# nrclaudio/spVIPES

Measured on AMD Instinct MI355X. Metric: cells/sec/training-step (2-group PoE VAE), higher is better.
Workload: dtype bf16

## Files before the change

include/spvipes_hip.h:

```cpp
#ifndef SPVIPES_HIP_H
#define SPVIPES_HIP_H

#include <stdint.h>

#ifdef __cplusplus
extern "C" {
#endif

#define SPV_OK 0
#define SPV_ERR_ARG (-1)
#define SPV_ERR_LAUNCH (-2)
#define SPV_ERR_UNSUPPORTED (-3)

#define SPV_COUNT_F32 0
#define SPV_COUNT_U16 1

#define SPV_NB_CMAX 64
#define SPV_DEC_KP 16
#define SPV_DEC_KS 32
#define SPV_DEC_KP_WIDE 32
#define SPV_DEC_KS_WIDE 64
#define SPV_DEC_CELLS_PER_WG 128

int spv_version(void);
// ... 252 lines not shown
  int32_t D;
  int32_t k;
  const int32_t* exclude;
  int32_t n_split;
  int32_t* idx; float* dist; int64_t ld_out;
  void* ws;
} spv_knn_args;
int spv_knn(const spv_knn_args* a, void* stream);
int32_t spv_knn_splits(int32_t n_q, int32_t n_c);
int64_t spv_knn_ws_bytes(int32_t n_q, int32_t k, int32_t n_split);
int32_t spv_knn_tile_q(void);
int32_t spv_knn_tile_c(void);

#define SPV_OT_DMAX 64
#define SPV_OT_KMAX 64
#define SPV_OT_SPLIT_MAX 64
typedef struct spv_ot_args {
  const float* Q; int64_t ld_q; int32_t n_q;
  const float* C; int64_t ld_c; int32_t n_c;
  int32_t D;
  int32_t k;
  const float* h;
  const float* r;
  float inv_eps;
  int32_t n_split;
  float* L;
  int32_t* idx; float* val; int64_t ld_out;
  float* mass;
  void* ws;
} spv_ot_args;
int spv_ot_softmin(const spv_ot_args* a, void* stream);
int spv_ot_topk(const spv_ot_args* a, void* stream);
int32_t spv_ot_splits(int32_t n_q, int32_t n_c);
int64_t spv_ot_ws_bytes(int32_t n_q, int32_t k, int32_t n_split);
int32_t spv_ot_tile_q(void);
int32_t spv_ot_tile_c(void);

#define SPV_OT_SEG_MAX 256
typedef struct spv_ot_seg_args {
  const float* Q; int64_t ld_q; int32_t n_q;
  const float* C; int64_t ld_c; int32_t n_c;
  int32_t D;
  const float* h;
  float inv_eps;
  const int32_t* seg_ptr; int32_t n_seg;
  int32_t n_split;
  float* L; int64_t ld_l;
  void* ws;
} spv_ot_seg_args;
int spv_ot_segment_lse(const spv_ot_seg_args* a, void* stream);
int32_t spv_ot_segment_splits(int32_t n_q, int32_t n_c);
int64_t spv_ot_segment_ws_bytes(int32_t n_q, int32_t n_seg, int32_t n_split);

#define SPV_SILHOUETTE_SEG_MAX 256
typedef struct spv_silhouette_args {
  const float* Q; int64_t ld_q; int32_t n_q;
  const float* C; int64_t ld_c; int32_t n_c;
  int32_t D;
  const int32_t* seg_ptr; int32_t n_seg;
  int32_t n_split;
  double* S; int64_t ld_s;
  void* ws;
} spv_silhouette_args;
int spv_silhouette_sums(const spv_silhouette_args* a, void* stream);
int32_t spv_silhouette_splits(int32_t n_q, int32_t n_c);
int64_t spv_silhouette_ws_bytes(int32_t n_q, int32_t n_seg, int32_t n_split);

int spv_dec_dz(const spv_dec_params* p, const float* Tp, const float* Ts, float* dz_part, void* stream);

int spv_dec_softmax_bwd(const spv_dec_params* p, const float* Tp, const float* Ts, float* dz_part, void* stream);
int spv_dec_heads_bwd(const spv_dec_params* p, const float* Tp, const float* Ts, float* dz_part, float* dw_part, void* stream);

#define SPV_ADAM_MAX_IMAGES 16
#define SPV_IMAGE_BF16 0
#define SPV_IMAGE_F16 1
typedef struct spv_adam_image {
  int64_t begin, count;
  int32_t cols, row_off, col_off, fmt;
  int64_t ld;
  uint16_t* dst;
  float scale; int32_t _pad;
} spv_adam_image;

int spv_adam_step_images(float* p, const float* g, float* m, float* v, int64_t n, float lr, float beta1, float beta2, float eps,
                         float weight_decay, float bc1, float bc2, float grad_scale, const spv_adam_image* images, int32_t n_images,
                         int64_t* step_counter, const int64_t* t_dev, double beta1_d, double beta2_d, void* stream);

typedef struct spv_gather_prob { const uint32_t* src; const int32_t* idx; uint32_t* dst; int64_t count; } spv_gather_prob;
int spv_gather_u32(const spv_gather_prob* probs, int32_t nprob, void* stream);

int spv_randn(float* out, int64_t n, const int64_t* counter, uint64_t key, void* stream);
int spv_counter_bump(int64_t* counter, void* stream);

int spv_adam_step(float* p, const float* g, float* m, float* v, int64_t n, float lr, float beta1,
                  float beta2, float eps, float weight_decay, float bc1, float bc2, float grad_scale,
                  void* stream);

#define SPV_MAXP 8

typedef struct spv_linear_prob {
  const float* X; int64_t ldx;
  const float* W;
  const float* bias;
  float* Y; int64_t ldy;
  const float* dY; int64_t lddy;
  float* dX; int64_t lddx;
  float* dW; float* db;
  int32_t N, K;
  const float* keep;
  const float* W2; int32_t n_w2;
  uint16_t* img_hi; uint16_t* img_lo; int64_t ld_img; int32_t img_rows;
} spv_linear_prob;
typedef struct spv_linear_batch {
  spv_linear_prob p[SPV_MAXP];
  int32_t nprob, B;
  int32_t relu;
  float drop_p;
  uint64_t seed;
  const uint64_t* seed_ptr;
  int32_t accumulate;
} spv_linear_batch;
int spv_linear_fwd(const spv_linear_batch* a, void* stream);
int spv_linear_dgrad(const spv_linear_batch* a, void* stream);
int spv_linear_wgrad(const spv_linear_batch* a, float* wpart, int64_t wpart_elems, void* stream);

typedef struct spv_linear_pending_prob { float* dW; float* db; int32_t N, K; } spv_linear_pending_prob;
typedef struct spv_linear_pending {
  spv_linear_pending_prob p[SPV_MAXP];
  int32_t nprob;
  const float* wpart; int64_t prob_stride;
} spv_linear_pending;
int spv_linear_bwd(const spv_linear_batch* d, const spv_linear_batch* w, float* wpart, int64_t wpart_elems,
                   const spv_linear_pending* pending, void* stream);
int spv_linear_reduce_pending(const spv_linear_pending* pending, void* stream);

typedef struct spv_bn_prob {
  const float* X; int64_t ldx;
  float* Y; int64_t ldy;
  const float* gamma; const float* beta;
  float* running_mean; float* running_var;
  float* stats;
  float* part;
  const float* dY; int64_t lddy;
  float* dX; int64_t lddx;
  float* dgamma; float* dbeta;
  int32_t N;
  uint16_t* img_hi; uint16_t* img_lo; int64_t ld_img; int32_t img_rows;
} spv_bn_prob;
typedef struct spv_bn_batch {
  spv_bn_prob p[SPV_MAXP];
  int32_t nprob, B, training, relu;
  float eps, momentum;
} spv_bn_batch;
int spv_bn_fwd(const spv_bn_batch* a, void* stream);
int spv_bn_bwd(const spv_bn_batch* a, void* stream);

typedef struct spv_sample_prob {
  const float* post; int32_t n;
  const float* eps;
  float* scale; float* logz; float* theta; float* kl;
  const float* g_loc; const float* g_logvar; const float* g_scale; const float* g_logz; const float* g_kl;
  float* d_post;
  int64_t g_ld;
} spv_sample_prob;
typedef struct spv_sample_batch { spv_sample_prob p[SPV_MAXP]; int32_t nprob, B; } spv_sample_batch;
int spv_enc_sample_fwd(const spv_sample_batch* a, void* stream);
int spv_enc_sample_bwd(const spv_sample_batch* a, void* stream);
int spv_enc_heads_fwd(const spv_bn_batch* bn, const spv_sample_batch* sb, void* stream);
int spv_enc_heads_bwd(const spv_bn_batch* bn, const spv_sample_batch* sb, void* stream);
// ... 45 lines not shown
} spv_poe_comp_args;
int spv_poe_comp_fwd(const spv_poe_comp_args* a, void* stream);
int spv_poe_comp_bwd(const spv_poe_comp_args* a, void* stream);

typedef struct spv_plan {
  const int32_t* ptr0; const int32_t* ind0; const float* val0; int32_t n0;
  const int32_t* ptr1; const int32_t* ind1; const float* val1; int32_t n1;
} spv_plan;
int spv_plan_invmap(const int32_t* idx0, int32_t B0, const int32_t* idx1, int32_t B1, int32_t* inv0, int32_t n0, int32_t* inv1,
                    int32_t n1, void* stream);
typedef struct spv_plan_expert_args {
  spv_plan plan;
  const int32_t* idx[2]; const int32_t* inv[2]; const float* comp[2];
  const float* stats[2]; int64_t ld[2];
  float* expert[2]; int64_t ld_expert[2];
  float* rowsum[2];
  const float* d_expert[2]; float* d_stats[2];
  int32_t B, n;
} spv_plan_expert_args;
int spv_plan_expert_fwd(const spv_plan_expert_args* a, void* stream);
int spv_plan_expert_bwd(const spv_plan_expert_args* a, void* stream);
int spv_plan_argmax(const spv_plan* plan, const int32_t* idx0, const int32_t* idx1, const int32_t* inv0, const int32_t* inv1,
                    int32_t B0, int32_t B1, int32_t* partner0, int32_t* partner1, void* stream);

typedef struct spv_zsplit_args {
  const float* priv[2]; const float* poe[2];
  float* zcat[2];
  const float* d_zcat[2]; float* d_priv[2]; float* d_poe[2];
  int32_t B, n_p, n_s, ngroups;
  uint16_t* am_hi[2]; uint16_t* am_lo[2]; int64_t ld_am; int32_t am_col; int32_t am_cols;
  uint16_t* aps_hi[2]; uint16_t* aps_lo[2]; int32_t Bp;
  int32_t kslots;
} spv_zsplit_args;
int spv_zsplit_fwd(const spv_zsplit_args* a, void* stream);
int spv_zsplit_bwd(const spv_zsplit_args* a, void* stream);

typedef struct spv_fold_prob {
  const float* W; const float* gamma; const float* beta;
  float* running_mean; float* running_var;
  const float* zsum; const float* zz;
  const float* z; int64_t ldz;
  float* stat;
  uint16_t* img_hi; uint16_t* img_lo; int64_t ld_img; int32_t col_off; int32_t slot;
  const float* dWeff; int64_t ld_dw;
  float* dW; float* dgamma; float* dbeta;
  float* red_part;
  float* dz; int64_t lddz;
  int32_t G, Gp, K;
  int32_t zcol; float* out_priv; float* out_poe; int32_t n_p, n_s;
} spv_fold_prob;
typedef struct spv_fold_batch {
  spv_fold_prob p[SPV_MAXP]; int32_t nprob, B, training; float eps, momentum;
  int32_t kslots;
} spv_fold_batch;
int spv_bn_fold_fwd(const spv_fold_batch* a, void* stream);
int spv_bn_fold_bwd(const spv_fold_batch* a, void* stream);

#define SPV_TRUNK_KMAX 48
typedef struct spv_trunk_prob {
  const float* W; const float* bias; const float* gamma; const float* beta;
  float* running_mean; float* running_var;
  const float* zsum; const float* zz;
  float* Wf; float* cf; float* stat;
  const float* dWf; const float* dcf;
  float* dW; float* dbias; float* dgamma; float* dbeta;
  float* dred;
  const float* z; int64_t ldz; float* dz; int64_t lddz;
  int32_t N, K;
} spv_trunk_prob;
typedef struct spv_trunk_batch { spv_trunk_prob p[2]; int32_t nprob, B, training; float eps, momentum; } spv_trunk_batch;
int spv_trunk_fold_fwd(const spv_trunk_batch* a, void* stream);
int spv_trunk_fold_bwd(const spv_trunk_batch* a, void* stream);

#define SPV_MAXR 16
typedef struct spv_reduce_prob {
  const float* src; int64_t slab_stride; int64_t ld_src; int32_t nslabs; int32_t col_off;
  int32_t rows, cols;
  float* dst; int64_t ld_dst; int32_t accumulate; int32_t pad_;
  const float* alpha; const float* exp_scale;
} spv_reduce_prob;
typedef struct spv_reduce_batch { spv_reduce_prob p[SPV_MAXR]; int32_t nprob; } spv_reduce_batch;
int spv_reduce_slabs(const spv_reduce_batch* b, void* stream);

int spv_loss_assemble(const float* rec0, const float* rec1, const float* w, const float* const* kl, int32_t nkl, int32_t B,
                      const float* kl_weight, float* loss, float* rec_sum, float* gkl, void* stream);

#ifdef __cplusplus
}
#endif
#endif
```

spvipes_amd/_abi.py:

```python
from __future__ import annotations

import ctypes as C
import os
from typing import NamedTuple, Optional

import torch

_HERE = os.path.dirname(os.path.abspath(__file__))
LIB_PATH = os.path.join(_HERE, "_lib", "libspvipes_hip.so")

SPV_COUNT_F32, SPV_COUNT_U16 = 0, 1
NB_CMAX, DEC_KP, DEC_KS, DEC_CELLS_PER_WG = 64, 16, 32, 128
DEC_KPS = DEC_KP + DEC_KS


class DecSlots(NamedTuple):
    kslots: int
    KP: int
    KS: int
    KPS: int


DEC_NARROW = DecSlots(0, DEC_KP, DEC_KS, DEC_KPS)
DEC_WIDE = DecSlots(1, 32, 64, 96)
# ... 46 lines not shown
                ("N", C.c_int32), ("K", C.c_int32), ("keep", C.c_void_p), ("W2", C.c_void_p), ("n_w2", C.c_int32),
                ("img_hi", C.c_void_p), ("img_lo", C.c_void_p), ("ld_img", C.c_int64), ("img_rows", C.c_int32)]


class SpvLinearBatch(C.Structure):
    _fields_ = [("p", SpvLinearProb * SPV_MAXP), ("nprob", C.c_int32), ("B", C.c_int32), ("relu", C.c_int32), ("drop_p", C.c_float),
                ("seed", C.c_uint64), ("seed_ptr", C.c_void_p), ("accumulate", C.c_int32)]


class SpvLinearPendingProb(C.Structure):
    _fields_ = [("dW", C.c_void_p), ("db", C.c_void_p), ("N", C.c_int32), ("K", C.c_int32)]


class SpvLinearPending(C.Structure):
    _fields_ = [("p", SpvLinearPendingProb * SPV_MAXP), ("nprob", C.c_int32), ("wpart", C.c_void_p), ("prob_stride", C.c_int64)]


class SpvBnProb(C.Structure):
    _fields_ = [("X", C.c_void_p), ("ldx", C.c_int64), ("Y", C.c_void_p), ("ldy", C.c_int64), ("gamma", C.c_void_p), ("beta", C.c_void_p),
                ("running_mean", C.c_void_p), ("running_var", C.c_void_p), ("stats", C.c_void_p), ("part", C.c_void_p),
                ("dY", C.c_void_p), ("lddy", C.c_int64), ("dX", C.c_void_p), ("lddx", C.c_int64), ("dgamma", C.c_void_p), ("dbeta", C.c_void_p),
                ("N", C.c_int32), ("img_hi", C.c_void_p), ("img_lo", C.c_void_p), ("ld_img", C.c_int64), ("img_rows", C.c_int32)]


class SpvBnBatch(C.Structure):
    _fields_ = [("p", SpvBnProb * SPV_MAXP), ("nprob", C.c_int32), ("B", C.c_int32), ("training", C.c_int32), ("relu", C.c_int32),
                ("eps", C.c_float), ("momentum", C.c_float)]


class SpvSampleProb(C.Structure):
    _fields_ = [("post", C.c_void_p), ("n", C.c_int32), ("eps", C.c_void_p), ("scale", C.c_void_p), ("logz", C.c_void_p), ("theta", C.c_void_p),
                ("kl", C.c_void_p), ("g_loc", C.c_void_p), ("g_logvar", C.c_void_p), ("g_scale", C.c_void_p), ("g_logz", C.c_void_p),
                ("g_kl", C.c_void_p), ("d_post", C.c_void_p), ("g_ld", C.c_int64)]


class SpvSampleBatch(C.Structure):
    _fields_ = [("p", SpvSampleProb * SPV_MAXP), ("nprob", C.c_int32), ("B", C.c_int32)]


class SpvPoeArgs(C.Structure):
    _fields_ = [("stats", C.c_void_p * 2), ("ld", C.c_int64 * 2), ("partner", C.c_void_p * 2), ("mode", C.c_void_p * 2), ("eps", C.c_void_p * 2),
                ("loc", C.c_void_p * 2), ("logvar", C.c_void_p * 2), ("scale", C.c_void_p * 2), ("logz", C.c_void_p * 2), ("theta", C.c_void_p * 2),
                ("kl", C.c_void_p * 2), ("g_loc", C.c_void_p * 2), ("g_logvar", C.c_void_p * 2), ("g_scale", C.c_void_p * 2),
                ("g_logz", C.c_void_p * 2), ("g_kl", C.c_void_p * 2), ("d_stats", C.c_void_p * 2), ("B", C.c_int32 * 2), ("n", C.c_int32),
                ("clamp_scale", C.c_int32), ("lone_passthrough", C.c_int32), ("expert", C.c_void_p * 2), ("ld_expert", C.c_int64 * 2),
                ("d_expert", C.c_void_p * 2), ("lab", C.c_void_p * 2), ("order", C.c_void_p * 2), ("rank", C.c_void_p * 2), ("tables", C.c_void_p)]


SPV_POE_MAXG, POE_COMP_SEG, POE_COMP_CMAX = 4, 16, 64


class SpvFc1FwdArgs(C.Structure):
    _fields_ = [("x", C.POINTER(SpvCounts)), ("B", C.c_int32), ("G", C.c_int32), ("W1_hi", C.c_void_p), ("W1_lo", C.c_void_p), ("ldw", C.c_int64),
                ("N1", C.c_int32), ("bias", C.c_void_p), ("bias2", C.c_void_p), ("n_first", C.c_int32), ("nsplit", C.c_int32), ("splits", C.c_int32),
                ("slabs", C.c_void_p), ("rowsum_ws", C.c_void_p), ("h1", C.c_void_p), ("library", C.c_void_p), ("xb_all", C.c_void_p),
                ("ld_xb", C.c_int64), ("library_all", C.c_void_p), ("cov", C.c_void_p), ("cov_idx", C.c_void_p)]


class SpvFc1BwdArgs(C.Structure):
    _fields_ = [("dh1", C.c_void_p), ("h1", C.c_void_p), ("x", C.POINTER(SpvCounts)), ("B", C.c_int32), ("G", C.c_int32), ("N1", C.c_int32),
                ("n_first", C.c_int32), ("nsplit", C.c_int32), ("Bp", C.c_int32), ("dh_hi", C.c_void_p), ("dh_lo", C.c_void_p), ("ld_dh", C.c_int64),
                ("part", C.c_void_p), ("db", C.c_void_p), ("db2", C.c_void_p), ("dW", C.c_void_p), ("dW2", C.c_void_p), ("ldc", C.c_int64),
                ("xb", C.c_void_p), ("ld_xb", C.c_int64), ("scale_ws", C.c_void_p)]


class SpvGatherProb(C.Structure):
    _fields_ = [("src", C.c_void_p), ("idx", C.c_void_p), ("dst", C.c_void_p), ("count", C.c_int64)]


def gather_u32(probs) -> None:
    arr = (SpvGatherProb * len(probs))()
    for a, (src, idx, dst) in zip(arr, probs):
        a.src, a.idx, a.dst, a.count = ptr(src), ptr(idx), ptr(dst), dst.numel()
    call("spv_gather_u32", arr, len(probs), stream_ptr())


ADAM_MAX_IMAGES = 16
IMAGE_BF16, IMAGE_F16 = 0, 1


class SpvAdamImage(C.Structure):
    _fields_ = [("begin", C.c_int64), ("count", C.c_int64), ("cols", C.c_int32), ("row_off", C.c_int32), ("col_off", C.c_int32), ("fmt", C.c_int32),
                ("ld", C.c_int64), ("dst", C.c_void_p), ("scale", C.c_float), ("_pad", C.c_int32)]


class SpvPoeCompArgs(C.Structure):
    _fields_ = ([("ngroups", C.c_int32), ("n", C.c_int32), ("ncomp", C.c_int32), ("pad_", C.c_int32), ("B", C.c_int32 * SPV_POE_MAXG),
                 ("stats", C.c_void_p * SPV_POE_MAXG), ("ld", C.c_int64 * SPV_POE_MAXG), ("comp", C.c_void_p * SPV_POE_MAXG),
                 ("eps", C.c_void_p * SPV_POE_MAXG), ("part", C.c_void_p), ("mean", C.c_void_p)]
                + [(k, C.c_void_p * SPV_POE_MAXG) for k in ("loc", "logvar", "scale", "logz", "theta", "kl", "g_loc", "g_logvar", "g_scale", "g_logz", "g_kl",
                                                            "dpn", "d_stats")])


class SpvPlan(C.Structure):
    _fields_ = [("ptr0", C.c_void_p), ("ind0", C.c_void_p), ("val0", C.c_void_p), ("n0", C.c_int32),
                ("ptr1", C.c_void_p), ("ind1", C.c_void_p), ("val1", C.c_void_p), ("n1", C.c_int32)]


class SpvPlanExpertArgs(C.Structure):
    _fields_ = [("plan", SpvPlan), ("idx", C.c_void_p * 2), ("inv", C.c_void_p * 2), ("comp", C.c_void_p * 2), ("stats", C.c_void_p * 2),
                ("ld", C.c_int64 * 2), ("expert", C.c_void_p * 2), ("ld_expert", C.c_int64 * 2), ("rowsum", C.c_void_p * 2),
                ("d_expert", C.c_void_p * 2), ("d_stats", C.c_void_p * 2), ("B", C.c_int32), ("n", C.c_int32)]


class SpvZsplitArgs(C.Structure):
    _fields_ = [("priv", C.c_void_p * 2), ("poe", C.c_void_p * 2), ("zcat", C.c_void_p * 2), ("d_zcat", C.c_void_p * 2),
                ("d_priv", C.c_void_p * 2), ("d_poe", C.c_void_p * 2), ("B", C.c_int32), ("n_p", C.c_int32), ("n_s", C.c_int32), ("ngroups", C.c_int32),
                ("am_hi", C.c_void_p * 2), ("am_lo", C.c_void_p * 2), ("ld_am", C.c_int64), ("am_col", C.c_int32), ("am_cols", C.c_int32),
                ("aps_hi", C.c_void_p * 2), ("aps_lo", C.c_void_p * 2), ("Bp", C.c_int32), ("kslots", C.c_int32)]


class SpvFoldProb(C.Structure):
    _fields_ = [("W", C.c_void_p), ("gamma", C.c_void_p), ("beta", C.c_void_p), ("running_mean", C.c_void_p), ("running_var", C.c_void_p),
                ("zsum", C.c_void_p), ("zz", C.c_void_p), ("z", C.c_void_p), ("ldz", C.c_int64), ("stat", C.c_void_p),
                ("img_hi", C.c_void_p), ("img_lo", C.c_void_p), ("ld_img", C.c_int64), ("col_off", C.c_int32), ("slot", C.c_int32),
                ("dWeff", C.c_void_p), ("ld_dw", C.c_int64), ("dW", C.c_void_p), ("dgamma", C.c_void_p), ("dbeta", C.c_void_p),
                ("red_part", C.c_void_p), ("dz", C.c_void_p), ("lddz", C.c_int64), ("G", C.c_int32), ("Gp", C.c_int32), ("K", C.c_int32),
                ("zcol", C.c_int32), ("out_priv", C.c_void_p), ("out_poe", C.c_void_p), ("n_p", C.c_int32), ("n_s", C.c_int32)]


class SpvFoldBatch(C.Structure):
    _fields_ = [("p", SpvFoldProb * SPV_MAXP), ("nprob", C.c_int32), ("B", C.c_int32), ("training", C.c_int32), ("eps", C.c_float),
                ("momentum", C.c_float), ("kslots", C.c_int32)]


class SpvGemmFixup(C.Structure):
    _fields_ = [("counters", C.c_void_p), ("alpha", C.c_void_p), ("dst0", C.c_void_p), ("ld0", C.c_int64), ("n0", C.c_int32),
                ("dst1", C.c_void_p), ("ld1", C.c_int64), ("c1", C.c_int32), ("n1", C.c_int32)]


class SpvGemmArgs(C.Structure):
    _fields_ = [("a_kmajor", C.c_int32), ("pad0_", C.c_int32), ("A_hi", C.c_void_p), ("A_lo", C.c_void_p), ("lda", C.c_int64),
                ("B_hi", C.c_void_p), ("B_lo", C.c_void_p), ("ldb", C.c_int64), ("C", C.c_void_p), ("ldc", C.c_int64),
                ("M", C.c_int32), ("N", C.c_int32), ("K", C.c_int32), ("nsplit", C.c_int32), ("splits", C.c_int32), ("a_tiles", C.c_int32),
                ("slab_stride", C.c_int64)]


class SpvDecGroup(C.Structure):
    _fields_ = [("p", SpvDecParams), ("library", C.c_void_p), ("px_r", C.c_void_p),
                ("Am_hi", C.c_void_p), ("Am_lo", C.c_void_p), ("Wm_hi", C.c_void_p), ("Wm_lo", C.c_void_p), ("K", C.c_int32), ("nsplit", C.c_int32),
                ("Tp", C.c_void_p), ("Ts", C.c_void_p), ("dz_part", C.c_void_p), ("dw_part", C.c_void_p)]


class SpvDecExpectedArgs(C.Structure):
    _fields_ = [("Am_hi", C.c_void_p), ("Am_lo", C.c_void_p), ("Wm_hi", C.c_void_p), ("Wm_lo", C.c_void_p), ("K", C.c_int32), ("nsplit", C.c_int32),
                ("genes", C.c_void_p), ("n_genes", C.c_int32), ("what", C.c_int32), ("out", C.c_void_p), ("ld_out", C.c_int64),
                ("alpha", C.c_float), ("accumulate", C.c_int32)]


class SpvDecSampleArgs(C.Structure):
    _fields_ = [("Am_hi", C.c_void_p), ("Am_lo", C.c_void_p), ("Wm_hi", C.c_void_p), ("Wm_lo", C.c_void_p), ("K", C.c_int32), ("nsplit", C.c_int32),
                ("genes", C.c_void_p), ("n_genes", C.c_int32), ("ld_gene", C.c_int32), ("theta", C.c_void_p), ("cell_ids", C.c_void_p),
                ("key", C.c_uint64), ("sample", C.c_uint32), ("out", C.c_void_p), ("ld_out", C.c_int64)]


class SpvDecSampleStatsArgs(C.Structure):
    _fields_ = [("Am_hi", C.c_void_p), ("Am_lo", C.c_void_p), ("Wm_hi", C.c_void_p), ("Wm_lo", C.c_void_p), ("K", C.c_int32), ("nsplit", C.c_int32),
                ("genes", C.c_void_p), ("n_genes", C.c_int32), ("n_seg", C.c_int32), ("theta", C.c_void_p), ("cell_ids", C.c_void_p),
                ("key", C.c_uint64), ("sample", C.c_uint32), ("seg", C.c_void_p), ("stats", C.c_void_p), ("ld_stats", C.c_int64),
                ("cell_total", C.c_void_p)]


class SpvDecExpectedStatsArgs(C.Structure):
    _fields_ = [("Am_hi", C.c_void_p), ("Am_lo", C.c_void_p), ("Wm_hi", C.c_void_p), ("Wm_lo", C.c_void_p), ("K", C.c_int32), ("nsplit", C.c_int32),
                ("genes", C.c_void_p), ("n_genes", C.c_int32), ("n_seg", C.c_int32), ("tile_seg", C.c_void_p), ("tile_n", C.c_void_p),
                ("stats", C.c_void_p), ("ld_stats", C.c_int64), ("ws", C.c_void_p)]
# ... 109 lines not shown
    "spv_dec_lse": (C.c_int, [C.POINTER(SpvDecParams), C.c_void_p, C.c_void_p]),
    "spv_dec_nb_fwd": (C.c_int, [C.POINTER(SpvDecParams), C.c_int32, C.c_void_p]),
    "spv_dec_logits": (C.c_int, [C.c_void_p, C.c_void_p, C.c_void_p, C.c_void_p, C.c_int32, C.c_int32, C.c_int32, C.c_int32,
                                 C.c_void_p, C.c_int32, C.c_void_p]),
    "spv_dec_materialize": (C.c_int, [C.POINTER(SpvDecParams), C.c_void_p, C.c_void_p, C.c_void_p, C.c_void_p, C.c_void_p, C.c_int64, C.c_void_p]),
    "spv_dec_expected": (C.c_int, [C.POINTER(SpvDecParams), C.POINTER(SpvDecExpectedArgs), C.c_void_p]),
    "spv_dec_sample": (C.c_int, [C.POINTER(SpvDecParams), C.POINTER(SpvDecSampleArgs), C.c_void_p]),
    "spv_dec_sample_stats": (C.c_int, [C.POINTER(SpvDecParams), C.POINTER(SpvDecSampleStatsArgs), C.c_void_p]),
    "spv_dec_expected_stats": (C.c_int, [C.POINTER(SpvDecParams), C.POINTER(SpvDecExpectedStatsArgs), C.c_void_p]),
    "spv_dec_expected_stats_ws_bytes": (C.c_int64, [C.c_int32, C.c_int32]),
    "spv_nbmix_sample": (C.c_int, [C.c_void_p, C.c_void_p, C.c_void_p, C.c_int64, C.c_void_p, C.c_int32, C.c_int32, C.c_void_p, C.c_uint64, C.c_uint32,
                                   C.c_void_p, C.c_int64, C.c_void_p]),
    "spv_de_pairs": (C.c_int, [C.POINTER(SpvDePairsArgs), C.c_void_p]),
    "spv_de_pairs_splits": (C.c_int32, [C.c_int32, C.c_int32]),
    "spv_de_median": (C.c_int, [C.POINTER(SpvDeMedianArgs), C.c_void_p]),
    "spv_de_median_ws_bytes": (C.c_int64, [C.c_int32, C.c_int32]),
    "spv_count_stats": (C.c_int, [C.POINTER(SpvCountStatsArgs), C.c_void_p]),
    "spv_count_stats_partial": (C.c_int, [C.POINTER(SpvCountStatsArgs), C.c_void_p]),
    "spv_count_stats_merge": (C.c_int, [C.POINTER(SpvCountStatsArgs), C.c_void_p]),
    "spv_count_stats_tile": (C.c_int32, []),
    "spv_count_stats_slab": (C.c_int32, []),
    "spv_count_stats_ws_bytes": (C.c_int64, [C.c_int32, C.c_int32]),
    "spv_count_totals": (C.c_int, [C.POINTER(SpvCounts), C.c_int32, C.c_int32, C.c_void_p, C.c_void_p]),
    "spv_csr_totals": (C.c_int, [C.c_void_p, C.c_void_p, C.c_void_p, C.c_int32, C.c_int32, C.c_int32, C.c_void_p, C.c_void_p]),
    "spv_knn": (C.c_int, [C.POINTER(SpvKnnArgs), C.c_void_p]),
    "spv_knn_splits": (C.c_int32, [C.c_int32, C.c_int32]),
    "spv_knn_ws_bytes": (C.c_int64, [C.c_int32, C.c_int32, C.c_int32]),
    "spv_knn_tile_q": (C.c_int32, []),
    "spv_knn_tile_c": (C.c_int32, []),
    "spv_ot_softmin": (C.c_int, [C.POINTER(SpvOtArgs), C.c_void_p]),
    "spv_ot_topk": (C.c_int, [C.POINTER(SpvOtArgs), C.c_void_p]),
    "spv_ot_splits": (C.c_int32, [C.c_int32, C.c_int32]),
    "spv_ot_ws_bytes": (C.c_int64, [C.c_int32, C.c_int32, C.c_int32]),
    "spv_ot_tile_q": (C.c_int32, []),
    "spv_ot_tile_c": (C.c_int32, []),
    "spv_ot_segment_lse": (C.c_int, [C.POINTER(SpvOtSegArgs), C.c_void_p]),
    "spv_ot_segment_splits": (C.c_int32, [C.c_int32, C.c_int32]),
    "spv_ot_segment_ws_bytes": (C.c_int64, [C.c_int32, C.c_int32, C.c_int32]),
    "spv_silhouette_sums": (C.c_int, [C.POINTER(SpvSilhouetteArgs), C.c_void_p]),
    "spv_silhouette_splits": (C.c_int32, [C.c_int32, C.c_int32]),
    "spv_silhouette_ws_bytes": (C.c_int64, [C.c_int32, C.c_int32, C.c_int32]),
    "spv_dec_dz": (C.c_int, [C.POINTER(SpvDecParams), C.c_void_p, C.c_void_p, C.c_void_p, C.c_void_p]),
    "spv_dec_softmax_bwd": (C.c_int, [C.POINTER(SpvDecParams), C.c_void_p, C.c_void_p, C.c_void_p, C.c_void_p]),
    "spv_dec_heads_bwd": (C.c_int, [C.POINTER(SpvDecParams), C.c_void_p, C.c_void_p, C.c_void_p, C.c_void_p, C.c_void_p]),
    "spv_dec_tables_grouped": (C.c_int, [C.POINTER(SpvDecGroup), C.c_int32, C.c_void_p]),
    "spv_dec_logits_grouped": (C.c_int, [C.POINTER(SpvDecGroup), C.c_int32, C.c_void_p]),
    "spv_dec_lse_grouped": (C.c_int, [C.POINTER(SpvDecGroup), C.c_int32, C.c_void_p]),
    "spv_dec_nb_fwd_grouped": (C.c_int, [C.POINTER(SpvDecGroup), C.c_int32, C.c_int32, C.c_void_p]),
    "spv_dec_heads_bwd_grouped": (C.c_int, [C.POINTER(SpvDecGroup), C.c_int32, C.c_void_p]),
    "spv_gemm_bf16_grouped": (C.c_int, [C.POINTER(SpvGemmArgs), C.c_int32, C.c_void_p]),
    "spv_linear_fwd": (C.c_int, [C.POINTER(SpvLinearBatch), C.c_void_p]),
    "spv_linear_dgrad": (C.c_int, [C.POINTER(SpvLinearBatch), C.c_void_p]),
    "spv_linear_wgrad": (C.c_int, [C.POINTER(SpvLinearBatch), C.c_void_p, C.c_int64, C.c_void_p]),
    "spv_linear_bwd": (C.c_int, [C.POINTER(SpvLinearBatch), C.POINTER(SpvLinearBatch), C.c_void_p, C.c_int64, C.POINTER(SpvLinearPending), C.c_void_p]),
    "spv_linear_reduce_pending": (C.c_int, [C.POINTER(SpvLinearPending), C.c_void_p]),
    "spv_bn_fwd": (C.c_int, [C.POINTER(SpvBnBatch), C.c_void_p]),
    "spv_bn_bwd": (C.c_int, [C.POINTER(SpvBnBatch), C.c_void_p]),
    "spv_enc_sample_fwd": (C.c_int, [C.POINTER(SpvSampleBatch), C.c_void_p]),
    "spv_enc_sample_bwd": (C.c_int, [C.POINTER(SpvSampleBatch), C.c_void_p]),
    "spv_enc_heads_fwd": (C.c_int, [C.POINTER(SpvBnBatch), C.POINTER(SpvSampleBatch), C.c_void_p]),
    "spv_enc_heads_bwd": (C.c_int, [C.POINTER(SpvBnBatch), C.POINTER(SpvSampleBatch), C.c_void_p]),
    "spv_poe_partner": (C.c_int, [C.c_void_p, C.c_void_p, C.c_int32, C.c_int32, C.c_void_p, C.c_void_p, C.c_void_p, C.c_void_p, C.c_void_p,
                                  C.c_void_p, C.c_void_p, C.c_void_p, C.c_void_p, C.c_void_p, C.c_void_p]),
    "spv_poe_rank": (C.c_int, [C.c_void_p, C.c_void_p, C.c_int32, C.c_int32, C.c_void_p, C.c_void_p, C.c_void_p, C.c_void_p, C.c_void_p, C.c_void_p, C.c_void_p]),
    "spv_poe_fuse_fwd": (C.c_int, [C.POINTER(SpvPoeArgs), C.c_void_p]),
    "spv_poe_fuse_bwd": (C.c_int, [C.POINTER(SpvPoeArgs), C.c_void_p]),
    "spv_plan_invmap": (C.c_int, [C.c_void_p, C.c_int32, C.c_void_p, C.c_int32, C.c_void_p, C.c_int32, C.c_void_p, C.c_int32, C.c_void_p]),
    "spv_plan_argmax": (C.c_int, [C.POINTER(SpvPlan), C.c_void_p, C.c_void_p, C.c_void_p, C.c_void_p, C.c_int32, C.c_int32, C.c_void_p,
                                  C.c_void_p, C.c_void_p]),
    "spv_plan_expert_fwd": (C.c_int, [C.POINTER(SpvPlanExpertArgs), C.c_void_p]),
    "spv_plan_expert_bwd": (C.c_int, [C.POINTER(SpvPlanExpertArgs), C.c_void_p]),
    "spv_poe_comp_fwd": (C.c_int, [C.POINTER(SpvPoeCompArgs), C.c_void_p]),
    "spv_poe_comp_bwd": (C.c_int, [C.POINTER(SpvPoeCompArgs), C.c_void_p]),
    "spv_zsplit_fwd": (C.c_int, [C.POINTER(SpvZsplitArgs), C.c_void_p]),
    "spv_zsplit_bwd": (C.c_int, [C.POINTER(SpvZsplitArgs), C.c_void_p]),
    "spv_bn_fold_fwd": (C.c_int, [C.POINTER(SpvFoldBatch), C.c_void_p]),
    "spv_bn_fold_bwd": (C.c_int, [C.POINTER(SpvFoldBatch), C.c_void_p]),
    "spv_trunk_fold_fwd": (C.c_int, [C.POINTER(SpvTrunkBatch), C.c_void_p]),
    "spv_trunk_fold_bwd": (C.c_int, [C.POINTER(SpvTrunkBatch), C.c_void_p]),
    "spv_reduce_slabs": (C.c_int, [C.POINTER(SpvReduceBatch), C.c_void_p]),
    "spv_loss_assemble": (C.c_int, [C.c_void_p, C.c_void_p, C.c_void_p, C.POINTER(C.c_void_p), C.c_int32, C.c_int32, C.c_void_p, C.c_void_p,
                                    C.c_void_p, C.c_void_p, C.c_void_p]),
    "spv_adam_step_images": (C.c_int, [C.c_void_p, C.c_void_p, C.c_void_p, C.c_void_p, C.c_int64, C.c_float, C.c_float, C.c_float, C.c_float,
                                       C.c_float, C.c_float, C.c_float, C.c_float, C.c_void_p, C.c_int32, C.c_void_p, C.c_void_p, C.c_double, C.c_double,
                                       C.c_void_p]),
    "spv_gather_u32": (C.c_int, [C.c_void_p, C.c_int32, C.c_void_p]),
    "spv_randn": (C.c_int, [C.c_void_p, C.c_int64, C.c_void_p, C.c_uint64, C.c_void_p]),
    "spv_counter_bump": (C.c_int, [C.c_void_p, C.c_void_p]),
    "spv_adam_step": (C.c_int, [C.c_void_p, C.c_void_p, C.c_void_p, C.c_void_p, C.c_int64, C.c_float, C.c_float, C.c_float,
                                C.c_float, C.c_float, C.c_float, C.c_float, C.c_float, C.c_void_p]),
}

EXPORTED_SYMBOLS = tuple(_SIGNATURES)
_lib = None


class SpvError(RuntimeError):
    pass


def load() -> C.CDLL:
    global _lib
    if _lib is not None:
        return _lib
    if not os.path.exists(LIB_PATH):
        raise SpvError(
            f"{LIB_PATH} is missing: build it with `python -m spvipes_amd.build` (hipcc, gfx950). "
            "spvipes_amd has no CPU or eager-PyTorch fallback for the hot path."
        )
    lib = C.CDLL(LIB_PATH)
    for name, (res, args) in _SIGNATURES.items():
        fn = getattr(lib, name)
        fn.restype, fn.argtypes = res, args
    from .build import build_id

    have, want = (lib.spv_build_id() or b"").decode(), build_id()
    if have != want and os.environ.get("SPV_ALLOW_STALE_LIB", "0") != "1":
        raise SpvError(f"{LIB_PATH} is stale (built from fingerprint {have}, the sources and flags now give {want}): "
                       "rebuild with `python -m spvipes_amd.build`")
    _lib = lib
    return lib


def check(rc: int, what: str) -> None:
    if rc != 0:
        msg = load().spv_last_error()
        raise SpvError(f"{what} failed with code {rc}: {msg.decode() if msg else ''}")


_PROFILE = None


def profile_start(names) -> None:
    global _PROFILE
    _PROFILE = {n: [] for n in names}


def profile_stop() -> dict:
    global _PROFILE
    prof, _PROFILE = _PROFILE or {}, None
    torch.cuda.synchronize()
    return {n: [s.elapsed_time(e) for s, e in evs] for n, evs in prof.items()}


def call(name: str, *args) -> None:
    fn = getattr(load(), name)
    if _PROFILE is not None and name in _PROFILE:
        s, e = torch.cuda.Event(enable_timing=True), torch.cuda.Event(enable_timing=True)
        s.record()
        rc = fn(*args)
        e.record()
        _PROFILE[name].append((s, e))
    else:
        rc = fn(*args)
    check(rc, name)


def stream_ptr() -> int:
    return torch.cuda.current_stream().cuda_stream


def ptr(t: Optional[torch.Tensor]) -> Optional[int]:
    if t is None:
        return None
    if not t.is_cuda:
        raise SpvError("spvipes_amd kernels need tensors resident in HBM (got a CPU tensor)")
    return t.data_ptr()

# ... 4 lines not shown
```

spvipes_amd/build.py:

```python
from __future__ import annotations

import os
import shutil
import subprocess
import sys

HERE = os.path.dirname(os.path.abspath(__file__))
CSRC = os.path.join(HERE, "csrc")
LIBDIR = os.path.join(HERE, "_lib")
LIB = os.path.join(LIBDIR, "libspvipes_hip.so")
SOURCES = ["spv_abi.hip"]
HEADERS = ["spv_common.h", "spv_gemm.h", "spv_fc1.h", "spv_dec_gemm.h", "spv_decoder.h", "spv_dec_expected.h", "spv_dec_sample.h", "spv_dec_sample_stats.h", "spv_dec_expected_stats.h", "spv_de.h", "spv_de_median.h", "spv_count_stats.h", "spv_knn.h", "spv_pair_scan.h", "spv_ot.h", "spv_ot_segments.h", "spv_silhouette.h", "spv_small.h", "spv_poe_n.h", os.path.join("..", "..", "include", "spvipes_hip.h")]


FLAGS = [
    "--offload-arch=gfx950", "-O3", "-std=c++17", "-fPIC", "-shared", "-Wno-unused-value",
    "-fno-slp-vectorize",
]


def build_id() -> str:
    import hashlib

    h = hashlib.sha256()
    h.update(" ".join(FLAGS).encode())
    for name in sorted(SOURCES + HEADERS):
        with open(os.path.join(CSRC, name), "rb") as f:
            h.update(name.replace(os.sep, "/").encode() + b"\0" + f.read())
    return h.hexdigest()[:32]


def _hipcc() -> str:
    for cand in (os.environ.get("HIPCC"), shutil.which("hipcc"), "/opt/rocm/bin/hipcc"):
        if cand and os.path.exists(cand):
            return cand
    raise RuntimeError("hipcc not found (need ROCm >= 7 with gfx950 support)")


def lib_build_id(path: str = LIB) -> str:
    import re

    if not os.path.exists(path):
        return ""
    with open(path, "rb") as f:
        m = re.search(rb"SPV_BUILD_ID=([0-9a-f]{32})", f.read())
    return m.group(1).decode() if m else ""


def is_stale() -> bool:
    return lib_build_id() != build_id()


def build(force: bool = False, verbose: bool = True) -> str:
    if not force and not is_stale():
        return LIB
    os.makedirs(LIBDIR, exist_ok=True)
    cmd = [
        _hipcc(), *FLAGS, f'-DSPV_BUILD_ID="{build_id()}"',
        *[os.path.join(CSRC, s) for s in SOURCES], "-o", LIB + ".tmp",
    ]
    if verbose:
        print("[spvipes_amd.build]", " ".join(cmd), flush=True)
    subprocess.run(cmd, check=True, cwd=CSRC)
    os.replace(LIB + ".tmp", LIB)
    return LIB


if __name__ == "__main__":
    build(force="--force" in sys.argv)
    print(LIB)
```

spvipes_amd/csrc/spv_abi.hip:

```cpp
#include "../../include/spvipes_hip.h"
#include "spv_common.h"
#include "spv_gemm.h"
#include "spv_fc1.h"
#include "spv_dec_gemm.h"
#include "spv_decoder.h"
#include "spv_dec_expected.h"
#include "spv_dec_sample.h"
#include "spv_dec_sample_stats.h"
#include "spv_dec_expected_stats.h"
#include "spv_de.h"
#include "spv_de_median.h"
#include "spv_count_stats.h"
#include "spv_knn.h"
#include "spv_ot.h"
#include "spv_ot_segments.h"
#include "spv_silhouette.h"
#include "spv_small.h"
#include "spv_poe_n.h"

#include <cstdio>
#include <cstdlib>
#include <cstring>
#include <type_traits>

// ... 1141 lines not shown
  if (dtype == SPV_COUNT_U16) hipLaunchKernelGGL((csr_totals_kernel<true>), grid, block, 0, (hipStream_t)stream, (const long*)indptr, cols, vals, n_cells, G, total);
  else if (dtype == SPV_COUNT_F32) hipLaunchKernelGGL((csr_totals_kernel<false>), grid, block, 0, (hipStream_t)stream, (const long*)indptr, cols, vals, n_cells, G, total);
  else return fail(SPV_ERR_ARG, "spv_csr_totals: unknown count dtype%s");
  return launch_status("spv_csr_totals");
}

extern "C" int spv_dec_dz(const spv_dec_params* q, const float* Tp, const float* Ts, float* dz_part, void* stream) {
  DecParams p;
  int rc = to_dec(q, p);
  if (rc != SPV_OK) return rc;
  if (!Tp || !Ts || !p.tP || !p.tS || !p.lse_p || !p.lse_s || !dz_part) return fail(SPV_ERR_ARG, "spv_dec_dz: null pointer%s");
  if (p.n_gene_tiles != p.Gp / 32) return fail(SPV_ERR_ARG, "spv_dec_dz: n_gene_tiles must be Gp / 32%s");
  if (p.grads_f32) return fail(SPV_ERR_UNSUPPORTED, "spv_dec_dz: needs bf16 gradient arrays%s");
  if (dec_kw(q) != 1) return fail(SPV_ERR_UNSUPPORTED, "spv_dec_dz: narrow operand layout only (kslots = 0)%s");
  hipLaunchKernelGGL((dec_softmax_bwd_kernel<bf16_t, true, false>), dim3(p.Bp / DEC_CELLS_PER_WG, p.gene_splits), dim3(256), 0, (hipStream_t)stream, p, Tp, Ts, dz_part, (float*)nullptr, (float*)nullptr);
  return launch_status("spv_dec_dz");
}

extern "C" int spv_dec_softmax_bwd(const spv_dec_params* q, const float* Tp, const float* Ts, float* dz_part, void* stream) {
  DecParams p;
  int rc = to_dec(q, p);
  if (rc != SPV_OK) return rc;
  if (!Tp || !Ts || !p.tP || !p.tS || !p.lse_p || !p.lse_s) return fail(SPV_ERR_ARG, "spv_dec_softmax_bwd: null pointer%s");
  if (p.n_gene_tiles != p.Gp / 32) return fail(SPV_ERR_ARG, "spv_dec_softmax_bwd: n_gene_tiles must be Gp / 32%s");
  dim3 grid(p.Bp / DEC_CELLS_PER_WG, p.gene_splits);
  hipStream_t s = (hipStream_t)stream;
  float* const none = nullptr;
  if (dec_kw(q) == 2) {
    if (dz_part) return fail(SPV_ERR_UNSUPPORTED, "spv_dec_softmax_bwd: the wide operand layout (kslots = 1) takes no dz_part%s");
    if (p.grads_f32) hipLaunchKernelGGL((dec_softmax_bwd_kernel<split_t, false, true, false, 2>), grid, dim3(256), 0, s, p, Tp, Ts, none, none, none);
    else hipLaunchKernelGGL((dec_softmax_bwd_kernel<bf16_t, false, true, false, 2>), grid, dim3(256), 0, s, p, Tp, Ts, none, none, none);
    return launch_status("spv_dec_softmax_bwd");
  }
  if (p.grads_f32 && dz_part) hipLaunchKernelGGL((dec_softmax_bwd_kernel<split_t, true>), grid, dim3(256), 0, s, p, Tp, Ts, dz_part, none, none);
  else if (p.grads_f32) hipLaunchKernelGGL((dec_softmax_bwd_kernel<split_t, false>), grid, dim3(256), 0, s, p, Tp, Ts, none, none, none);
  else if (dz_part) hipLaunchKernelGGL((dec_softmax_bwd_kernel<bf16_t, true>), grid, dim3(256), 0, s, p, Tp, Ts, dz_part, none, none);
  else hipLaunchKernelGGL((dec_softmax_bwd_kernel<bf16_t, false>), grid, dim3(256), 0, s, p, Tp, Ts, none, none, none);
  return launch_status("spv_dec_softmax_bwd");
}

static int heads_bwd_prepare(const spv_dec_params* q, const float* Tp, const float* Ts, const float* dz_part, const float* dw_part, DecParams& p) {
  int rc = to_dec(q, p);
  if (rc != SPV_OK) return rc;
  if (!Tp || !Ts || !p.tP || !p.tS || !p.lse_p || !p.lse_s || !dz_part || !dw_part) return fail(SPV_ERR_ARG, "spv_dec_heads_bwd: null pointer%s");
  if (p.n_gene_tiles != p.Gp / 32) return fail(SPV_ERR_ARG, "spv_dec_heads_bwd: n_gene_tiles must be Gp / 32%s");
  if (p.Bp % DEC_CELLS_PER_WG) return fail(SPV_ERR_ARG, "spv_dec_heads_bwd: Bp must be a multiple of 128%s");
  if (p.grads_f32 && (!p.Wps_lo || !p.Aps_lo)) return fail(SPV_ERR_ARG, "spv_dec_heads_bwd: split gradient words need the lo planes of the operand images%s");
  if (dec_kw(q) != 1) return fail(SPV_ERR_UNSUPPORTED, "spv_dec_heads_bwd: narrow operand layout only (kslots = 0)%s");
  return SPV_OK;
}
extern "C" int spv_dec_heads_bwd(const spv_dec_params* q, const float* Tp, const float* Ts, float* dz_part, float* dw_part, void* stream) {
  DecParams p;
  int rc = heads_bwd_prepare(q, Tp, Ts, dz_part, dw_part, p);
  if (rc != SPV_OK) return rc;
  dim3 grid(p.Bp / DEC_CELLS_PER_WG, p.gene_splits);
  if (p.grads_f32) {
    launch_lds<dec_heads_bwd_split_kernel>(grid, dim3(256), HBS_LDS_BYTES, (hipStream_t)stream, p, Tp, Ts, dz_part, dw_part);
    return launch_status("spv_dec_heads_bwd");
  }
  hipLaunchKernelGGL(dec_heads_bwd_kernel, grid, dim3(256), 0, (hipStream_t)stream, p, Tp, Ts, dz_part, dw_part);
  return launch_status("spv_dec_heads_bwd");
}
extern "C" int spv_dec_heads_bwd_grouped(const spv_dec_group* g, int32_t n, void* stream) {
  if (!g || n <= 0) return fail(SPV_ERR_ARG, "spv_dec_heads_bwd_grouped: bad arguments%s");
  return pairs_then_rest(n,
    [&](int i) {
      HeadsBwdArgs a0, a1;
      int rc = heads_bwd_prepare(&g[i].p, g[i].Tp, g[i].Ts, g[i].dz_part, g[i].dw_part, a0.p);
      if (rc != SPV_OK) return rc;
      rc = heads_bwd_prepare(&g[i + 1].p, g[i + 1].Tp, g[i + 1].Ts, g[i + 1].dz_part, g[i + 1].dw_part, a1.p);
      if (rc != SPV_OK) return rc;
      if (a0.p.grads_f32 || a1.p.grads_f32) return NOT_A_PAIR;
      a0.Tp = g[i].Tp; a0.Ts = g[i].Ts; a0.dz_part = g[i].dz_part; a0.dw_part = g[i].dw_part;
      a1.Tp = g[i + 1].Tp; a1.Ts = g[i + 1].Ts; a1.dz_part = g[i + 1].dz_part; a1.dw_part = g[i + 1].dw_part;
      hipLaunchKernelGGL(dec_heads_bwd_pair_kernel, dim3(max2(a0.p.Bp, a1.p.Bp) / DEC_CELLS_PER_WG, max2(a0.p.gene_splits, a1.p.gene_splits), 2), dim3(256), 0, (hipStream_t)stream, a0, a1);
      return launch_status("spv_dec_heads_bwd_grouped");
    },
    [&](int i) { return spv_dec_heads_bwd(&g[i].p, g[i].Tp, g[i].Ts, g[i].dz_part, g[i].dw_part, stream); });
}

__global__ void adam_kernel(float* __restrict__ p, const float* __restrict__ g, float* __restrict__ m, float* __restrict__ v,
                            long n, float lr, float b1, float b2, float eps, float wd, float bc1, float bc2, float gscale) {
  const long stride = (long)gridDim.x * blockDim.x * 4;
  const float step = lr / bc1, isq = rsqrtf(bc2);
  for (long i = ((long)blockIdx.x * blockDim.x + threadIdx.x) * 4; i < n; i += stride) {
    if (i + 4 <= n) {
      f4v pp = *reinterpret_cast<f4v*>(p + i), gg = *reinterpret_cast<const f4v*>(g + i);
      f4v mm = *reinterpret_cast<f4v*>(m + i), vv = *reinterpret_cast<f4v*>(v + i);
#pragma unroll
      for (int j = 0; j < 4; ++j) {
        const float gr = gg[j] * gscale + wd * pp[j];
        mm[j] = b1 * mm[j] + (1.f - b1) * gr;
        vv[j] = b2 * vv[j] + (1.f - b2) * gr * gr;
        pp[j] -= step * mm[j] / (sqrtf(vv[j]) * isq + eps);
      }
      *reinterpret_cast<f4v*>(p + i) = pp; *reinterpret_cast<f4v*>(m + i) = mm; *reinterpret_cast<f4v*>(v + i) = vv;
    } else {
      for (long k = i; k < n; ++k) {
        const float gr = g[k] * gscale + wd * p[k];
        m[k] = b1 * m[k] + (1.f - b1) * gr;
        v[k] = b2 * v[k] + (1.f - b2) * gr * gr;
        p[k] -= step * m[k] / (sqrtf(v[k]) * isq + eps);
      }
    }
  }
}

struct GatherBatch { int n; spv_gather_prob p[SPV_MAXP]; };
__global__ __launch_bounds__(256) void gather_u32_kernel(GatherBatch a) {
  const spv_gather_prob& q = a.p[blockIdx.y];
  const long i = (long)blockIdx.x * 256 + threadIdx.x;
  if (i < q.count) q.dst[i] = q.src[q.idx ? (long)q.idx[i] : i];
}
extern "C" int spv_gather_u32(const spv_gather_prob* probs, int32_t nprob, void* stream) {
  if (!probs || nprob <= 0 || nprob > SPV_MAXP) return fail(SPV_ERR_ARG, "spv_gather_u32: bad arguments%s");
  GatherBatch a{};
  a.n = nprob;
  long nmax = 0;
  for (int i = 0; i < nprob; ++i) {
    if (!probs[i].src || !probs[i].dst || probs[i].count < 0) return fail(SPV_ERR_ARG, "spv_gather_u32: bad problem%s");
    a.p[i] = probs[i];
    nmax = probs[i].count > nmax ? probs[i].count : nmax;
  }
  if (nmax == 0) return SPV_OK;
  hipLaunchKernelGGL(gather_u32_kernel, dim3((unsigned)((nmax + 255) / 256), nprob), dim3(256), 0, (hipStream_t)stream, a);
  return launch_status("spv_gather_u32");
}

__global__ __launch_bounds__(256) void randn_kernel(float* __restrict__ out, long n, const long long* __restrict__ counter, unsigned long long key) {
  const long i4 = ((long)blockIdx.x * blockDim.x + threadIdx.x) * 4;
  if (i4 >= n) return;
  const unsigned long long step = counter ? (unsigned long long)*counter : 0ull;
  unsigned c[4] = {(unsigned)(i4 >> 2), (unsigned)((unsigned long long)(i4 >> 2) >> 32), (unsigned)step, (unsigned)(step >> 32)};
  const unsigned k[2] = {(unsigned)key, (unsigned)(key >> 32)};
  philox4x32_10(c, k);
  float z[4];
#pragma unroll
  for (int h = 0; h < 2; ++h) {
    const float u1 = ((float)(c[2 * h] >> 8) + 0.5f) * (1.0f / 16777216.0f);
    const float u2 = ((float)(c[2 * h + 1] >> 8) + 0.5f) * (1.0f / 16777216.0f);
    const float rad = sqrtf(-2.0f * __logf(u1));
    float sn, cs;
    __sincosf(6.283185307179586f * u2, &sn, &cs);
    z[2 * h] = rad * cs; z[2 * h + 1] = rad * sn;
  }
  if (i4 + 4 <= n && ((reinterpret_cast<uintptr_t>(out + i4) & 15) == 0)) *reinterpret_cast<f4v*>(out + i4) = f4v{z[0], z[1], z[2], z[3]};
  else for (int j = 0; j < 4 && i4 + j < n; ++j) out[i4 + j] = z[j];
}
__global__ void counter_bump_kernel(long long* counter) { if (threadIdx.x == 0 && blockIdx.x == 0) *counter += 1; }

extern "C" int spv_counter_bump(int64_t* counter, void* stream) {
  if (!counter) return fail(SPV_ERR_ARG, "spv_counter_bump: null counter%s");
  hipLaunchKernelGGL(counter_bump_kernel, dim3(1), dim3(64), 0, (hipStream_t)stream, (long long*)counter);
  return launch_status("spv_counter_bump");
}

extern "C" int spv_randn(float* out, int64_t n, const int64_t* counter, uint64_t key, void* stream) {
  if (!out || n < 0) return fail(SPV_ERR_ARG, "spv_randn: bad arguments%s");
  if (n == 0) return SPV_OK;
  hipLaunchKernelGGL(randn_kernel, dim3((unsigned)((n + 1023) / 1024)), dim3(256), 0, (hipStream_t)stream, out, (long)n, (const long long*)counter, (unsigned long long)key);
  return launch_status("spv_randn");
}

struct AdamImages { int n; spv_adam_image img[SPV_ADAM_MAX_IMAGES]; };

__global__ void adam_images_kernel(float* __restrict__ p, const float* __restrict__ g, float* __restrict__ m, float* __restrict__ v,
                                   long n, float lr, float b1, float b2, float eps, float wd, float bc1, float bc2, float gscale, AdamImages im,
                                   long long* step_counter, const long long* t_dev, double b1d, double b2d) {
  if (step_counter && blockIdx.x == 0 && threadIdx.x == 0) *step_counter += 1;
  if (t_dev) {
    long long e = *t_dev + 1;
    double r1 = 1.0, r2 = 1.0, x1 = b1d, x2 = b2d;
    while (e > 0) { if (e & 1) { r1 *= x1; r2 *= x2; } x1 *= x1; x2 *= x2; e >>= 1; }
    bc1 = (float)(1.0 - r1); bc2 = (float)(1.0 - r2);
  }
  const long stride = (long)gridDim.x * blockDim.x * 4;
  const float step = lr / bc1, isq = rsqrtf(bc2);
  for (long i = ((long)blockIdx.x * blockDim.x + threadIdx.x) * 4; i < n; i += stride) {
    float out[4];
    const int cnt = (i + 4 <= n) ? 4 : (int)(n - i);
    if (cnt == 4) {
      f4v pp = *reinterpret_cast<f4v*>(p + i), gg = *reinterpret_cast<const f4v*>(g + i);
      f4v mm = *reinterpret_cast<f4v*>(m + i), vv = *reinterpret_cast<f4v*>(v + i);
#pragma unroll
      for (int j = 0; j < 4; ++j) {
        const float gr = gg[j] * gscale + wd * pp[j];
        mm[j] = b1 * mm[j] + (1.f - b1) * gr;
        vv[j] = b2 * vv[j] + (1.f - b2) * gr * gr;
        pp[j] -= step * mm[j] / (sqrtf(vv[j]) * isq + eps);
        out[j] = pp[j];
      }
      *reinterpret_cast<f4v*>(p + i) = pp; *reinterpret_cast<f4v*>(m + i) = mm; *reinterpret_cast<f4v*>(v + i) = vv;
    } else {
      for (int j = 0; j < cnt; ++j) {
        const long k = i + j;
        const float gr = g[k] * gscale + wd * p[k];
        m[k] = b1 * m[k] + (1.f - b1) * gr;
        v[k] = b2 * v[k] + (1.f - b2) * gr * gr;
        p[k] -= step * m[k] / (sqrtf(v[k]) * isq + eps);
        out[j] = p[k];
      }
    }
    for (int d = 0; d < im.n; ++d) {
      const spv_adam_image& q = im.img[d];
      const long k0 = i - q.begin;
      if (k0 + cnt <= 0 || k0 >= q.count) continue;
      const unsigned cols = (unsigned)q.cols;
      unsigned r = (unsigned)k0 / cols, c = (unsigned)k0 - r * cols;
      uint16_t* dst = q.dst + ((long)r + q.row_off) * q.ld + q.col_off;
      const bool half = q.fmt == SPV_IMAGE_F16;
      if (cnt == 4 && k0 + 4 <= q.count && c + 4 <= cols && (((reinterpret_cast<uintptr_t>(dst + c)) & 7) == 0)) {
        typedef __attribute__((ext_vector_type(4))) unsigned short us4;
        *reinterpret_cast<us4*>(dst + c) = half ? us4{f2h(out[0] * q.scale), f2h(out[1] * q.scale), f2h(out[2] * q.scale), f2h(out[3] * q.scale)}
                                                : us4{f2bf(out[0]), f2bf(out[1]), f2bf(out[2]), f2bf(out[3])};
      } else {
        for (int j = 0; j < cnt && k0 + j < q.count; ++j) {
          dst[c] = half ? f2h(out[j] * q.scale) : f2bf(out[j]);
          if (++c == cols) { c = 0; dst += q.ld; }
        }
      }
      break;
    }
  }
}

extern "C" int spv_adam_step_images(float* p, const float* g, float* m, float* v, int64_t n, float lr, float beta1, float beta2, float eps,
                                    float weight_decay, float bc1, float bc2, float grad_scale, const spv_adam_image* images, int32_t n_images,
                                    int64_t* step_counter, const int64_t* t_dev, double beta1_d, double beta2_d, void* stream) {
  if (!p || !g || !m || !v || n < 0 || n_images < 0 || n_images > SPV_ADAM_MAX_IMAGES || (n_images && !images)) return fail(SPV_ERR_ARG, "spv_adam_step_images: bad arguments%s");
  if (n == 0) return SPV_OK;
  if ((reinterpret_cast<uintptr_t>(p) | reinterpret_cast<uintptr_t>(g) | reinterpret_cast<uintptr_t>(m) | reinterpret_cast<uintptr_t>(v)) & 15)
    return fail(SPV_ERR_ARG, "spv_adam_step_images: buffers must be 16-byte aligned%s");
  AdamImages im{};
  im.n = n_images;
  for (int d = 0; d < n_images; ++d) {
    const spv_adam_image& q = images[d];
    if (!q.dst || q.begin < 0 || (q.begin & 3) || q.count <= 0 || q.begin + q.count > n || q.cols <= 0 || q.ld < q.cols + q.col_off || q.row_off < 0 || q.col_off < 0 ||
        q.count >= (1L << 31) || (q.fmt != SPV_IMAGE_BF16 && q.fmt != SPV_IMAGE_F16) || (q.fmt == SPV_IMAGE_F16 && !(q.scale > 0.f)))
      return fail(SPV_ERR_ARG, "spv_adam_step_images: bad image descriptor%s");
    im.img[d] = q;
  }
  long blocks = (n / 4 + 255) / 256;
  if (blocks > 2048) blocks = 2048;
  if (blocks < 1) blocks = 1;
  hipLaunchKernelGGL(adam_images_kernel, dim3((unsigned)blocks), dim3(256), 0, (hipStream_t)stream, p, g, m, v, (long)n, lr, beta1, beta2, eps,
                     weight_decay, bc1, bc2, grad_scale, im, (long long*)step_counter, (const long long*)t_dev, beta1_d, beta2_d);
  return launch_status("spv_adam_step_images");
}

extern "C" int spv_adam_step(float* p, const float* g, float* m, float* v, int64_t n, float lr, float beta1, float beta2,
                             float eps, float weight_decay, float bc1, float bc2, float grad_scale, void* stream) {
  if (!p || !g || !m || !v || n < 0) return fail(SPV_ERR_ARG, "spv_adam_step: bad arguments%s");
  if (n == 0) return SPV_OK;
  if ((reinterpret_cast<uintptr_t>(p) | reinterpret_cast<uintptr_t>(g) | reinterpret_cast<uintptr_t>(m) | reinterpret_cast<uintptr_t>(v)) & 15)
    return fail(SPV_ERR_ARG, "spv_adam_step: buffers must be 16-byte aligned%s");
  long blocks = (n / 4 + 255) / 256;
  if (blocks > 2048) blocks = 2048;
  if (blocks < 1) blocks = 1;
  hipLaunchKernelGGL(adam_kernel, dim3((unsigned)blocks), dim3(256), 0, (hipStream_t)stream, p, g, m, v, (long)n, lr, beta1, beta2, eps,
                     weight_decay, bc1, bc2, grad_scale);
  return launch_status("spv_adam_step");
}

static int check_linear(const spv_linear_batch* a, const char* who) {
  if (!a || a->nprob <= 0 || a->nprob > SPV_MAXP || a->B <= 0) return fail(SPV_ERR_ARG, "%s: bad batch", who);
  if (a->drop_p < 0.f || a->drop_p >= 1.f) return fail(SPV_ERR_ARG, "%s: dropout probability outside [0,1)", who);
  for (int i = 0; i < a->nprob; ++i)
    if (a->p[i].N <= 0 || a->p[i].K <= 0 || !a->p[i].W) return fail(SPV_ERR_ARG, "%s: bad problem", who);
  return SPV_OK;
}
static void linear_extents(const spv_linear_batch* a, int& nmax, int& kmax) {
  nmax = kmax = 0;
  for (int i = 0; i < a->nprob; ++i) { nmax = a->p[i].N > nmax ? a->p[i].N : nmax; kmax = a->p[i].K > kmax ? a->p[i].K : kmax; }
}

extern "C" int spv_linear_fwd(const spv_linear_batch* a, void* stream) {
  int rc = check_linear(a, "spv_linear_fwd");
  if (rc) return rc;
  for (int i = 0; i < a->nprob; ++i) if (!a->p[i].X || !a->p[i].Y) return fail(SPV_ERR_ARG, "spv_linear_fwd: null pointer%s");
  int nmax, kmax; linear_extents(a, nmax, kmax);
  int rows = a->B;
  for (int i = 0; i < a->nprob; ++i) {
    const spv_linear_prob& q = a->p[i];
    if (q.img_hi && (q.ld_img < q.N || q.img_rows < 0)) return fail(SPV_ERR_ARG, "spv_linear_fwd: bad operand image%s");
    if (q.img_hi && q.img_rows > rows) rows = q.img_rows;
  }
  hipLaunchKernelGGL(linear_fwd_kernel, dim3((rows + 63) / 64, (nmax + 63) / 64, a->nprob), dim3(256), 0, (hipStream_t)stream, *a);
  return launch_status("spv_linear_fwd");
}
static int check_linear_dgrad(const spv_linear_batch* a, const char* who) {
  int rc = check_linear(a, who);
  if (rc) return rc;
  for (int i = 0; i < a->nprob; ++i)
    if (!a->p[i].dY || !a->p[i].dX || ((a->relu || a->drop_p > 0.f) && !a->p[i].Y)) return fail(SPV_ERR_ARG, "%s: null pointer", who);
  return SPV_OK;
}
static int check_linear_wgrad(const spv_linear_batch* a, const char* who) {
  int rc = check_linear(a, who);
  if (rc) return rc;
  for (int i = 0; i < a->nprob; ++i)
    if (!a->p[i].dY || !a->p[i].X || !a->p[i].dW || ((a->relu || a->drop_p > 0.f) && !a->p[i].Y)) return fail(SPV_ERR_ARG, "%s: null pointer", who);
  return SPV_OK;
}
static int check_linear_wpart(const spv_linear_batch* a, const float* wpart, int64_t wpart_elems, const char* who, int& nmax, int& kmax, long& prob_stride) {
  if (!wpart) return fail(SPV_ERR_ARG, "%s: workspace missing", who);
  linear_extents(a, nmax, kmax);
  prob_stride = (long)WG_SLICES * nmax * (kmax + 1);
  if (wpart_elems < prob_stride * a->nprob) return fail(SPV_ERR_ARG, "%s: workspace too small", who);
  return SPV_OK;
}

extern "C" int spv_linear_dgrad(const spv_linear_batch* a, void* stream) {
  int rc = check_linear_dgrad(a, "spv_linear_dgrad");
  if (rc) return rc;
  int nmax, kmax; linear_extents(a, nmax, kmax);
  hipLaunchKernelGGL(linear_dgrad_kernel, dim3((a->B + 63) / 64, (kmax + 63) / 64, a->nprob), dim3(256), 0, (hipStream_t)stream, *a);
  return launch_status("spv_linear_dgrad");
}
extern "C" int spv_linear_wgrad(const spv_linear_batch* a, float* wpart, int64_t wpart_elems, void* stream) {
  int nmax, kmax;
  long prob_stride;
  int rc = check_linear_wgrad(a, "spv_linear_wgrad");
  if (rc == SPV_OK) rc = check_linear_wpart(a, wpart, wpart_elems, "spv_linear_wgrad", nmax, kmax, prob_stride);
  if (rc) return rc;
  hipStream_t s = (hipStream_t)stream;
  if (a->B <= WG_DIRECT_MAX_B) {
    hipLaunchKernelGGL(linear_wgrad_direct_kernel, dim3((nmax + 31) / 32, (kmax + 31) / 32, a->nprob), dim3(256), 0, s, *a);
    return launch_status("spv_linear_wgrad");
  }
  hipLaunchKernelGGL(linear_wgrad_kernel, dim3((nmax + 31) / 32, (kmax + 31) / 32, a->nprob * WG_SLICES), dim3(256), 0, s, *a, wpart, prob_stride);
// ... 943 lines not shown
```

spvipes_amd/csrc/spv_small.h:

```cpp
#pragma once
#include "../../include/spvipes_hip.h"
#include "spv_common.h"

namespace spv {


typedef spv_linear_prob LinearProb;
typedef spv_linear_batch LinearBatch;

__device__ __forceinline__ unsigned hash_u32(unsigned long long x) {
  x ^= x >> 33; x *= 0xff51afd7ed558ccdULL; x ^= x >> 33; x *= 0xc4ceb9fe1a85ec53ULL; x ^= x >> 33;
  return (unsigned)x;
}
__device__ __forceinline__ bool dropout_keep(unsigned long long seed, int prob, long idx, float p) {
  const unsigned key = ((unsigned)seed ^ ((unsigned)(seed >> 32) * 0x9E3779B9u)) + (unsigned)(prob + 1) * 0x85EBCA6Bu;
  unsigned x = (unsigned)idx * 747796405u + key;
  x = ((x >> ((x >> 28) + 4u)) ^ x) * 277803737u;
  x ^= x >> 22;
  x = x * 0x2C1B3C6Du + key;
  x ^= x >> 15;
  return (float)(x >> 8) * (1.0f / 16777216.0f) >= p;
}

__device__ __forceinline__ f16v mfma_f32(float x, float w, const f16v& c) { return __builtin_amdgcn_mfma_f32_32x32x2f32(x, w, c, 0, 0, 0); }

template <bool VEC>
__device__ __forceinline__ void load8(const float* p, const float* safe, int lim, float (&v)[8]) {
  if constexpr (VEC) {
    const float* s = (lim >= 8) ? p : safe;
    const f4v a = *reinterpret_cast<const f4v*>(s), b = *reinterpret_cast<const f4v*>(s + 4);
#pragma unroll
    for (int j = 0; j < 4; ++j) { v[j] = (lim >= 8) ? a[j] : 0.f; v[4 + j] = (lim >= 8) ? b[j] : 0.f; }
  } else {
#pragma unroll
    for (int j = 0; j < 8; ++j) { const float t = *((j < lim) ? p + j : safe); v[j] = (j < lim) ? t : 0.f; }
  }
}
__device__ __forceinline__ void load8_strided(const float* p, long ld, int c0, int lim, float (&v)[8]) {
#pragma unroll
  for (int j = 0; j < 8; ++j) { const bool ok = c0 + j < lim; const float t = p[ok ? (long)(c0 + j) * ld : 0]; v[j] = ok ? t : 0.f; }
}
__device__ __forceinline__ bool aligned16(const void* p) { return (reinterpret_cast<uintptr_t>(p) & 15) == 0; }

template <bool VX, bool VW>
__device__ __forceinline__ void linear_fwd_body(const LinearBatch& a) {
  const LinearProb& q = a.p[blockIdx.z];
  const int lane = threadIdx.x & 63, wave = threadIdx.x >> 6, h = lane >> 5, r = lane & 31;
  const int b0 = blockIdx.x * 64 + 32 * (wave >> 1), n0 = blockIdx.y * 64 + 32 * (wave & 1);
  const int rows_out = (q.img_hi != nullptr && q.img_rows > a.B) ? q.img_rows : a.B;
  if (n0 >= q.N || b0 >= rows_out) return;
  const int row = b0 + r, col = n0 + r;
  const float* xr = q.X + (long)min(row, a.B - 1) * q.ldx;
  const float* wr = q.W + (long)min(col, q.N - 1) * q.K;
  f16v acc;
#pragma unroll
  for (int i = 0; i < 16; ++i) acc[i] = 0.f;
  float xa[8], wb[8];
  load8<VX>(xr + 8 * h, xr, q.K - 8 * h, xa);
  load8<VW>(wr + 8 * h, wr, q.K - 8 * h, wb);
  for (int k0 = 0; k0 < q.K; k0 += 16) {
    float xn[8], wn[8];
    const int kn = k0 + 16 + 8 * h;
    load8<VX>(xr + kn, xr, q.K - kn, xn);
    load8<VW>(wr + kn, wr, q.K - kn, wn);
#pragma unroll
    for (int j = 0; j < 8; ++j) acc = mfma_f32(xa[j], wb[j], acc);
#pragma unroll
    for (int j = 0; j < 8; ++j) { xa[j] = xn[j]; wb[j] = wn[j]; }
  }
  if (col >= q.N) return;
  const float bias = q.bias ? q.bias[col] : 0.f;
#pragma unroll
  for (int i = 0; i < 16; ++i) {
    const int b = b0 + crow(i, h);
    if (b >= rows_out) continue;
    if (b >= a.B) {
      q.img_hi[(long)b * q.ld_img + col] = 0;
      if (q.img_lo != nullptr) q.img_lo[(long)b * q.ld_img + col] = 0;
      continue;
    }
    float v = acc[i] + bias;
    if (a.relu) v = fmaxf(v, 0.f);
    if (a.drop_p > 0.f) {
      const bool keep = q.keep ? (q.keep[(long)b * q.N + col] != 0.f)
                               : dropout_keep(a.seed + (a.seed_ptr ? *a.seed_ptr : 0ull), blockIdx.z, (long)b * q.N + col, a.drop_p);
// ... 1446 lines not shown
  float acc = v[0];
#pragma unroll
  for (int k = 1; k < NS; ++k) acc += v[k];
  return acc;
}
template <int NS, int V, bool EXTRA>
__device__ __forceinline__ void reduce_few_slabs(const spv_reduce_prob& q, float alpha) {
  const unsigned cols_v = (unsigned)q.cols / V, total = (unsigned)q.rows * cols_v;
  for (unsigned i = blockIdx.x * 256u + threadIdx.x; i < total; i += gridDim.x * 256u) {
    const unsigned r = i / cols_v, c = (i - r * cols_v) * V;
    const float* s = q.src + (long)r * q.ld_src + q.col_off + c;
    float* d = q.dst + (long)r * q.ld_dst + c;
    RedVec<V> v[NS];
#pragma unroll
    for (int k = 0; k < NS; ++k) v[k] = red_ld<V>(s + (long)k * q.slab_stride);
    RedVec<V> e, prev, out;
    if constexpr (EXTRA) {
      e = red_ld<V>(q.exp_scale ? q.exp_scale + c : g_spv_zero4);
      prev = red_ld<V>(q.accumulate ? d : g_spv_zero4);
    }
#pragma unroll
    for (int j = 0; j < V; ++j) {
      float t[NS];
#pragma unroll
      for (int k = 0; k < NS; ++k) t[k] = v[k].x[j];
      float a = reduce_ordered_sum<NS>(t) * alpha;
      if constexpr (EXTRA) {
        if (q.exp_scale) a *= expf(e.x[j]);
        a = q.accumulate ? prev.x[j] + a : a;
      }
      out.x[j] = a;
    }
    red_st(d, out);
  }
}
template <int V, bool EXTRA>
__device__ __forceinline__ void reduce_few_dispatch(const spv_reduce_prob& q, float alpha) {
  switch (q.nslabs) {
    case 1: reduce_few_slabs<1, V, EXTRA>(q, alpha); break;
    case 2: reduce_few_slabs<2, V, EXTRA>(q, alpha); break;
    case 3: reduce_few_slabs<3, V, EXTRA>(q, alpha); break;
    case 4: reduce_few_slabs<4, V, EXTRA>(q, alpha); break;
    case 5: reduce_few_slabs<5, V, EXTRA>(q, alpha); break;
    case 6: reduce_few_slabs<6, V, EXTRA>(q, alpha); break;
    case 7: reduce_few_slabs<7, V, EXTRA>(q, alpha); break;
    default: reduce_few_slabs<8, V, EXTRA>(q, alpha); break;
  }
}
__host__ __device__ inline long reduce_blocks_needed(const spv_reduce_prob& q) {
  const long total = (long)q.rows * q.cols;
  if (q.nslabs > RED_FEW_MAX) return (total + 63) / 64;
  return reduce_vec4(q) ? (total / 4 + 255) / 256 : (total + 255) / 256;
}
__global__ __launch_bounds__(256) void reduce_slabs_kernel(spv_reduce_batch b) {
  __shared__ float s_part[4][64];
  const spv_reduce_prob& q = b.p[blockIdx.y];
  const long total = (long)q.rows * q.cols;
  const float alpha = *(q.alpha ? q.alpha : &g_spv_one);
  if (q.nslabs <= RED_FEW_MAX) {
    const bool extra = q.exp_scale || q.accumulate;
    if (reduce_vec4(q)) { if (extra) reduce_few_dispatch<4, true>(q, alpha); else reduce_few_dispatch<4, false>(q, alpha); }
    else { if (extra) reduce_few_dispatch<1, true>(q, alpha); else reduce_few_dispatch<1, false>(q, alpha); }
    return;
  }
  const int tx = threadIdx.x & 63, ty = threadIdx.x >> 6;
  for (long base = (long)blockIdx.x * 64; base < total; base += (long)gridDim.x * 64) {
    const long i = base + tx;
    const bool ok = i < total;
    int r = 0, c = 0;
    float acc = 0.f;
    if (ok) {
      r = (int)(i / q.cols); c = (int)(i - (long)r * q.cols);
      const float* s = q.src + (long)r * q.ld_src + q.col_off + c;
#pragma unroll 8
      for (int k = ty; k < q.nslabs; k += 4) acc += s[(long)k * q.slab_stride];
    }
    s_part[ty][tx] = acc;
    __syncthreads();
    if (ty == 0 && ok) reduce_finish(q, r, c, ((s_part[0][tx] + s_part[1][tx]) + s_part[2][tx]) + s_part[3][tx], alpha);
    __syncthreads();
  }
}

__global__ __launch_bounds__(1024) void loss_assemble_kernel(const float* rec0, const float* rec1, const float* w, const float* kl0,
                                                             const float* kl1, const float* kl2, const float* kl3, int B,
                                                             const float* kl_weight, float* loss, float* rec_sum, float* gkl) {
  __shared__ float s_r[1024], s_k[1024];
  const int t = threadIdx.x;
  float ar = 0.f, ak = 0.f;
  const float klw = kl_weight ? *kl_weight : 1.f;
  const float gk = klw / (float)B;
  for (int i = t; i < B; i += 1024) {
    const float wi = w[i];
    ar += wi * rec0[i];
    ar += wi * ld_or_zero(rec1, i);
    float k = 0.f;
    k += ld_or_zero(kl0, i);
    k += ld_or_zero(kl1, i);
    k += ld_or_zero(kl2, i);
    k += ld_or_zero(kl3, i);
    ak += k;
    if (gkl) gkl[i] = gk;
  }
  s_r[t] = ar; s_k[t] = ak;
  __syncthreads();
  for (int o = 512; o > 0; o >>= 1) {
    if (t < o) { s_r[t] += s_r[t + o]; s_k[t] += s_k[t + o]; }
    __syncthreads();
  }
  if (t == 0) {
    if (rec_sum) *rec_sum = s_r[0];
    *loss = s_r[0] + gk * s_k[0];
  }
}

}
```

spvipes_amd/dec_ops.py:

```python
from __future__ import annotations

import ctypes as C
from typing import List, Optional, Sequence

import numpy as np
import torch

from . import _abi
from ._abi import (DEC_CELLS_PER_WG, DEC_NARROW, NB_CMAX, TRUNK_KMAX, SpvBnBatch, SpvDecExpectedArgs, SpvDecExpectedStatsArgs, SpvDecGroup, SpvDecSampleArgs, SpvDecSampleStatsArgs, SpvDecParams, SpvFoldBatch, SpvGemmArgs, SpvReduceBatch, SpvTrunkBatch, SpvZsplitArgs,
                   ptr, round_up, stream_ptr)
from .nn_ops import _add_lin, _first_ws, _fptr, _lin_batch, _linear_bwd, _reduce_pending, _wgrad, grad_out
from . import ops as _ops
from .ops import N_HIDDEN_MIX, GroupCounts, Workspace, _bf16_image, _gemm_slabs, _gene_splits, _nb_cell_tiles, _nb_splits, _pack, fork, group_streams, join

N_DEC_PARAMS = 13
KMP = 320


def _cont(t: torch.Tensor) -> torch.Tensor:
    return t if (t.is_contiguous() and t.dtype == torch.float32) else t.contiguous().float()


def _theta(par) -> torch.Tensor:
    return torch.exp(_cont(par[12]))


def dec_slots(decoder):
    return getattr(decoder, "dec_slots", DEC_NARROW)


def _slab_cols(KP: int, KS: int):
    return [(0, KP, 0, 0)] + [(KP + c, 32, 1, c) for c in range(0, KS, 32)]


def decoder_params(dec, px_r) -> List[torch.Tensor]:
    fp, fs, tr, mx = dec.factor_regressor_private, dec.factor_regressor_shared, dec.sigmoid_decoder, dec.mixture
    return [fp.linear.weight, fp.bn.weight, fp.bn.bias, fs.linear.weight, fs.bn.weight, fs.bn.bias,
            tr.linear.weight, tr.linear.bias, tr.bn.weight, tr.bn.bias, mx.linear.weight, mx.linear.bias, px_r]


def _add_red(b: SpvReduceBatch, src: torch.Tensor, nslabs: int, slab_stride: int, ld_src: int, rows: int, cols: int, dst: torch.Tensor,
             ld_dst: int, *, col_off: int = 0, dst_col: int = 0, accumulate: bool = False, alpha=None, exp_scale=None) -> None:
    q = b.p[b.nprob]
    q.src, q.slab_stride, q.ld_src, q.nslabs, q.col_off, q.rows, q.cols = ptr(src), slab_stride, ld_src, nslabs, col_off, rows, cols
    q.dst, q.ld_dst, q.accumulate = dst.data_ptr() + 4 * dst_col, ld_dst, int(accumulate)
    q.alpha, q.exp_scale = ptr(alpha), ptr(exp_scale)
    b.nprob += 1


def _add_heads_red(red: SpvReduceBatch, st: "_DecoderBwd", slabs, dWp: torch.Tensor, dWs: torch.Tensor, sl, alpha) -> None:
    G, KP, KS, KPS = st.G, sl.KP, sl.KS, sl.KPS
    if sl.kslots:
        for slab, n, hd, c0 in slabs:
            _add_red(red, slab, st.csp_n, G * n, n, G, n, (dWp, dWs)[hd], (KP, KS)[hd], dst_col=c0, alpha=alpha)
    elif st.fused_heads:
        _add_red(red, slabs[0], st.csp_n, st.Gp * KPS, KPS, G, KP, dWp, KP, alpha=alpha)
        _add_red(red, slabs[1], st.csp_n, st.Gp * KPS, KPS, G, KS, dWs, KS, col_off=KP, alpha=alpha)
    else:
        _add_red(red, slabs[0], st.csp_n, G * KP, KP, G, KP, dWp, KP, alpha=alpha)
        _add_red(red, slabs[1], st.csp_n, G * KS, KS, G, KS, dWs, KS, alpha=alpha)


def _run_red(b: SpvReduceBatch) -> None:
    if b.nprob:
        _abi.call("spv_reduce_slabs", C.byref(b), stream_ptr())


def _zsplit_args(B: int, Bp: int, n_p: int, n_s: int, n_m: int, sl, lat, zcat, Am_img, Aps_img) -> SpvZsplitArgs:
    za = SpvZsplitArgs()
    za.B, za.n_p, za.n_s, za.ngroups, za.kslots = B, n_p, n_s, len(lat), sl.kslots
    za.ld_am, za.am_col, za.am_cols, za.Bp = KMP, n_m, KMP - n_m, Bp
    for g, (pz, qz) in enumerate(lat):
        za.priv[g], za.poe[g], za.zcat[g] = ptr(pz), ptr(qz), ptr(zcat[g])
        za.am_hi[g], za.am_lo[g], za.aps_hi[g], za.aps_lo[g] = ptr(Am_img[g][0]), ptr(Am_img[g][1]), ptr(Aps_img[g][0]), ptr(Aps_img[g][1])
    return za


def _zstats_batch(B: int, n_p: int, n_s: int, zcat, zsum, zz, trunk=None):
    nt = n_p + n_s
    b = _lin_batch(B)
    for g, z in enumerate(zcat):
        for k, (off, n) in enumerate(((0, n_p), (n_p, n_s))):
            _add_lin(b, N=n, K=n, W=ptr(zz[g][k]), X=_fptr(z, off), ldx=nt, dY=_fptr(z, off), lddy=nt, dW=ptr(zz[g][k]), db=ptr(zsum[g][k]))
        if trunk is not None:
            _add_lin(b, N=nt, K=nt, W=ptr(trunk[1][g]), X=ptr(z), ldx=nt, dY=ptr(z), lddy=nt, dW=ptr(trunk[1][g]), db=ptr(trunk[0][g]))
    return b


def _fold_batch(B: int, training: bool, momentum: float, sl) -> SpvFoldBatch:
    fb = SpvFoldBatch()
    fb.nprob, fb.B, fb.training, fb.eps, fb.momentum, fb.kslots = 0, B, int(training), 1e-3, momentum, sl.kslots
    return fb


def _add_fold(fb: SpvFoldBatch, decoder, par, n_p: int, n_s: int, zcat, zsum, zz, fstat, Wps, G: int, Gp: int, sl) -> None:
    for k, (reg, W, gam, bet, off, slot, n, zoff) in enumerate(((decoder.factor_regressor_private, par[0], par[1], par[2], 0, sl.KP, n_p, 0),
                                                                (decoder.factor_regressor_shared, par[3], par[4], par[5], sl.KP, sl.KS, n_s, n_p))):
        q = fb.p[fb.nprob]
        q.W, q.gamma, q.beta, q.running_mean, q.running_var = ptr(W), ptr(gam), ptr(bet), ptr(reg.bn.running_mean), ptr(reg.bn.running_var)
        q.zsum, q.zz, q.z, q.ldz, q.stat = ptr(zsum[k]), ptr(zz[k]), _fptr(zcat, zoff), n_p + n_s, ptr(fstat[k])
        q.img_hi, q.img_lo, q.ld_img, q.col_off, q.slot = ptr(Wps[0]), ptr(Wps[1]), sl.KPS, off, slot
        q.G, q.Gp, q.K = G, Gp, n
        fb.nprob += 1


def _trunk_bn_batch(B: int, training: bool, momentum: float, decoders, par, pre_a, m, tstat, parts, n_m: int, Am_img=None, Bp: int = 0,
                    grads=None) -> SpvBnBatch:
    bn = SpvBnBatch()
    bn.nprob, bn.B, bn.training, bn.relu, bn.eps, bn.momentum = len(decoders), B, int(training), 1, 1e-3, momentum
    for g, dec in enumerate(decoders):
        tb = dec.sigmoid_decoder.bn
        q = bn.p[g]
        q.X, q.ldx, q.Y, q.ldy, q.gamma, q.beta = ptr(pre_a[g]), n_m, ptr(m[g]), n_m, ptr(par[g][8]), ptr(par[g][9])
        q.running_mean, q.running_var, q.stats, q.N = ptr(tb.running_mean), ptr(tb.running_var), ptr(tstat[g]), n_m
        q.part = ptr(parts[g])
        if Am_img is not None:
            q.img_hi, q.img_lo, q.ld_img, q.img_rows = ptr(Am_img[g][0]), ptr(Am_img[g][1]), KMP, Bp
        if grads is not None:
            q.dY, q.lddy, q.dX, q.lddx, q.dgamma, q.dbeta = ptr(grads[0][g]), n_m, ptr(grads[1][g]), n_m, ptr(grads[2][g]), ptr(grads[3][g])
    return bn


def _trunk_batch(B: int, training: bool, decoders, Wa, par, zsum_t, zz_t, Wf, cf, tstat, n_m: int, nt: int, bwd=None) -> SpvTrunkBatch:
    tb_ = SpvTrunkBatch()
    tb_.nprob, tb_.B, tb_.training, tb_.eps, tb_.momentum = len(decoders), B, int(training), 1e-3, 0.01
    for g, dec in enumerate(decoders):
        bnm = dec.sigmoid_decoder.bn
        q = tb_.p[g]
        q.W, q.bias, q.gamma, q.beta = ptr(Wa[g]), ptr(par[g][7]), ptr(par[g][8]), ptr(par[g][9])
        q.running_mean, q.running_var = ptr(bnm.running_mean), ptr(bnm.running_var)
        q.zsum, q.zz, q.Wf, q.cf, q.stat, q.N, q.K = ptr(zsum_t[g]), ptr(zz_t[g]), ptr(Wf[g]), ptr(cf[g]), ptr(tstat[g]), n_m, nt
        if bwd is not None:
            q.dWf, q.dcf, q.dW, q.dbias, q.dgamma, q.dbeta, q.dred, q.z, q.dz = (ptr(t) for t in bwd[g])
            q.ldz, q.lddz = nt, nt
    return tb_


def _dec_params(wsg: Workspace, pre: str, B: int, G: int, Bp: int, Gp: int, mlo: bool, sl, logits, Wps, Aps, *, cst=None, tabs=(None, None),
                w_row=None, nb=None, grads=None, grads_f32: bool = False, split_Bp: Optional[int] = None) -> SpvDecParams:
    splits, per = _gene_splits(split_Bp or Bp, Gp)
    nbs, nbper, nbtiles = nb if nb is not None else (1, 32, 0)
    vec = lambda nme: ptr(wsg.get(pre + nme, (Bp,), torch.float32))
    part = lambda nme: ptr(wsg.get(pre + nme, (splits, Bp), torch.float32))
    nbpart = lambda nme: ptr(wsg.get(pre + nme, (nbs, Bp), torch.float32)) if nb is not None else None
    dth, dL, tP, tS = grads if grads is not None else (None,) * 4
    counts = dict(X=cst.X, ldx=cst.ld, rows=cst.rows, col_off=cst.col_off, count_is_u16=int(cst.dtype == _abi.SPV_COUNT_U16)) if cst is not None else {}
    return SpvDecParams(
        B=B, G=G, Bp=Bp, Gp=Gp, logits=ptr(logits), n_gene_tiles=Gp // 32, logits_f32=int(mlo),
# ... 406 lines not shown
            ga = (SpvGemmArgs * NG)()
            outs = [stages[g].gemm_args(which, ga[g]) for g in range(NG)]
            _abi.call("spv_gemm_bf16_grouped", ga, NG, stream_ptr())
            return outs

        def pair_heads_bwd():
            hg = (SpvDecGroup * NG)()
            for g in range(NG):
                st = stages[g]
                hg[g].p, hg[g].Tp, hg[g].Ts, hg[g].dz_part, hg[g].dw_part = st.P, ptr(st.S["Tp"]), ptr(st.S["Ts"]), ptr(st.dz_part), ptr(st.dw_part)
            _abi.call("spv_dec_heads_bwd_grouped", hg, NG, stream_ptr())

        if pair:
            streams = [cur] * NG
            if not da_first:
                pair_heads_bwd()
            d_slabs = pair_gemm("d")
        fork(streams)
        for g in range(0 if pair else NG):
            with torch.cuda.stream(streams[g]):
                if not da_first:
                    stages[g].softmax()
                d_slabs[g] = stages[g].gemm_d()
                if not stages[g].fused_dz:
                    ef_slabs[g] = stages[g].gemm_ef()
        join(streams)
        side.wait_stream(cur)
        if da_first:
            with torch.cuda.stream(side):
                if pair:
                    pair_heads_bwd()
                else:
                    for st in stages:
                        st.softmax()
                sm_done = torch.cuda.Event()
                sm_done.record(side)
        al = g_loss
        for g in range(NG):
            st, G, Gp = stages[g], Gs[g], Gps[g]
            _add_red(red, d_slabs[g], st.ksp_m, B * KMP, KMP, B, n_m, dAm[g], n_m, alpha=al)
            _add_red(red, d_slabs[g], st.ksp_m, B * KMP, KMP, B, nt, d_zcat[g], nt, col_off=n_m, alpha=al)
            if st.fused_dz:
                _add_red(red2, st.dz_part, st.P.gene_splits, Bp * DEC_KPS, DEC_KPS, B, n_p, d_zcat[g], nt, accumulate=True, alpha=al)
                _add_red(red2, st.dz_part, st.P.gene_splits, Bp * DEC_KPS, DEC_KPS, B, n_s, d_zcat[g], nt, col_off=DEC_KP, dst_col=n_p, accumulate=True, alpha=al)
            elif sl.kslots:
                for slab, n, hd, c0 in ef_slabs[g]:
                    cols = min(n, (n_p, n_s)[hd] - c0)
                    if cols > 0:
                        _add_red(red2, slab, st.ksp_n, B * n, n, B, cols, d_zcat[g], nt, dst_col=(0, n_p)[hd] + c0, accumulate=True, alpha=al)
            else:
                _add_red(red2, ef_slabs[g][0], st.ksp_n, B * DEC_KP, DEC_KP, B, n_p, d_zcat[g], nt, accumulate=True, alpha=al)
                _add_red(red2, ef_slabs[g][1], st.ksp_n, B * DEC_KS, DEC_KS, B, n_s, d_zcat[g], nt, dst_col=n_p, accumulate=True, alpha=al)
            _add_red(red, ctx.saved_g[g]["dth"], -(-(Bp // 64) // _nb_cell_tiles(Bp, Gp)), Gp, Gp, 1, G, pg[g][12][0], G, alpha=al, exp_scale=par[g][12])
        gk = None
        if ctx.n_kl:
            gk = new(B)
            _add_red(red2, ctx.gkl, 1, B, B, 1, B, gk, B, alpha=g_loss)
        _run_red(red)
        if not da_first:
            _run_red(red2)
        bc_done = None
        with torch.cuda.stream(side):
            red_bc = SpvReduceBatch()
            red_bc.nprob = 0
            for g in range(NG):
                _add_heads_red(red_bc, stages[g], stages[g].gemm_bc(), dWp[g], dWs[g], sl, g_loss)
            _run_red(red_bc)
            if side is not cur:
                bc_done = torch.cuda.Event()
                bc_done.record(side)

        def issue_wm(after=None):
            with torch.cuda.stream(side):
                if after is not None:
                    side.wait_event(after)
                red3 = SpvReduceBatch()
                red3.nprob = 0
                wm_slabs = pair_gemm("a") if pair else None
                for g in range(NG):
                    st, G = stages[g], Gs[g]
                    a = wm_slabs[g] if pair else st.gemm_a()
                    _add_red(red3, a, st.csp_m, G * KMP, KMP, G, KM - 1, pg[g][10][0], KM - 1, alpha=g_loss)
                    _add_red(red3, a, st.csp_m, G * KMP, KMP, G, 1, pg[g][11][0], 1, col_off=KM - 1, alpha=g_loss)
                _run_red(red3)
            if _ops.DEFER_JOIN:
                _ops.defer(side, [g_loss])
            else:
                cur.wait_stream(side)

        if not wm_late:
            issue_wm()
        held = _trunk_bwd(r, [ctx.decoders[g] for g in range(NG)], par, training, ws, pg, dAm, d_zcat)

        def joins():
            if da_first:
                cur.wait_event(sm_done)
                _run_red(red2)
            if bc_done is not None:
                cur.wait_event(bc_done)
            if wm_late:
                ev = torch.cuda.Event()
                ev.record(cur)
                issue_wm(ev)

        d_priv, d_poe = _fold_bwd(r, training, ws, pg, dWp, dWs, d_zcat, joins)
        grads = [t for g in range(NG) for t in (d_priv[g], d_poe[g])] + [pg[g][j][1] for g in range(NG) for j in range(N_DEC_PARAMS)]
        return (None,) * 11 + tuple(grads) + (gk,) * ctx.n_kl


@torch.no_grad()
def _prepare_decoder(decoder, px_r: torch.Tensor, private_log_z: torch.Tensor, poe_log_z: torch.Tensor, library: torch.Tensor,
                     training: bool, nsplit: int, ws: Workspace, par=None, *, logits: bool, split_rows: Optional[int] = None) -> _DecOperands:
    par = list(par) if par is not None else decoder_params(decoder, px_r)
    pz, qz = _cont(private_log_z), _cont(poe_log_z)
    B, G, n_m, mlo = pz.shape[0], par[0].shape[0], par[6].shape[0], nsplit == 3
    r = _DecFront(private_log_z.device, B, [G], pz.shape[1], qz.shape[1], n_m, dec_slots(decoder), mlo)
    _front_latents(r, [(pz, qz)], [ws], "mat_")
    _front_zstats(r, training, False, [ws])
    _front_fold(r, [decoder], [par], training, 0.0, [ws], "mat_")
    _run_fold(r)
    r.Wm = [_front_wm(r, 0, par, ws, "mat_", reuse=False)]
    r.pre_a, r.m, r.tstat = [r.new(B, n_m)], [r.new(B, n_m)], [r.new(n_m, 2)]
    _front_trunk(r, [decoder], [par], training, False, 0.0, [ws], "mat_bn_part")
    Bp, Gp, (Am_hi, Am_lo), (Wm_hi, Wm_lo) = r.Bp, r.Gps[0], r.Am[0], r.Wm[0]
    tiled = None
    if logits:
        tiled = ws.get("mat_logits_" + ("f32" if mlo else "f16"), (Bp, Gp), torch.float32 if mlo else torch.float16)
        _abi.call("spv_dec_logits", ptr(Am_hi), ptr(Am_lo), ptr(Wm_hi), ptr(Wm_lo), KMP, Bp, Gp, nsplit, ptr(tiled), int(mlo), stream_ptr())
    p = _dec_params(ws, "mat_", B, G, Bp, Gp, mlo, r.sl, tiled, r.Wps[0], r.Aps[0], split_Bp=None if split_rows is None else round_up(int(split_rows), DEC_CELLS_PER_WG))
    lib = _cont(library.flatten())
    if lib.numel() != B:
        raise _abi.SpvError("decoder: the library vector must hold one value per cell")
    _abi.call("spv_dec_lse", C.byref(p), ptr(lib), stream_ptr())
    o = _DecOperands()
    o.p, o.B, o.G, o.Bp, o.Gp, o.Am, o.Wm, o.par, o.keep = p, B, G, Bp, Gp, r.Am[0], r.Wm[0], par, (pz, qz, lib)
    return o


@torch.no_grad()
def materialize_decoder(decoder, px_r: torch.Tensor, private_log_z: torch.Tensor, poe_log_z: torch.Tensor, library: torch.Tensor,
                        training: bool, nsplit: int, ws: Workspace, par=None) -> dict:
    o = _prepare_decoder(decoder, px_r, private_log_z, poe_log_z, library, training, nsplit, ws, par, logits=True)
    B, G = o.B, o.G
    new = lambda *s: torch.empty(*s, dtype=torch.float32, device=private_log_z.device)
    out = {k: new(B, G) for k in ("px_scale_private", "px_scale_shared", "px_rate_private", "px_rate_shared", "px_mixing")}
    _abi.call("spv_dec_materialize", C.byref(o.p), ptr(out["px_scale_private"]), ptr(out["px_scale_shared"]), ptr(out["px_rate_private"]),
              ptr(out["px_rate_shared"]), ptr(out["px_mixing"]), G, stream_ptr())
    out["px_r"] = _theta(o.par)
    return out


def _gene_selection(genes, G: int, dev, who: str):
    if genes is None:
        gidx, n = None, G
    elif isinstance(genes, torch.Tensor) and genes.is_cuda:
        if genes.dtype != torch.int32 or genes.dim() != 1 or not genes.is_contiguous():
            raise _abi.SpvError(f"{who}: a device gene list must be a contiguous 1-d int32 tensor")
        gidx, n = genes, int(genes.numel())
    else:
        host = np.asarray(genes.cpu() if isinstance(genes, torch.Tensor) else genes)
        if host.ndim != 1 or (host.size and not np.issubdtype(host.dtype, np.integer)):
            raise TypeError(f"{who}: genes must be a 1-d sequence of integer gene positions")
        bad = np.nonzero((host < 0) | (host >= G))[0]
        if bad.size:
            raise IndexError(f"gene position {int(host[bad[0]])} is out of range for a group of {G} genes")
        gidx, n = torch.as_tensor(host.astype(np.int32), device=dev), int(host.size)
    if n <= 0:
# ... 187 lines not shown
```

spvipes_amd/ops.py:

```python
from __future__ import annotations

import ctypes as C
import os
from dataclasses import dataclass
from typing import Dict, NamedTuple, Optional, Sequence, Tuple

import torch

from . import _abi
from ._abi import DEC_CELLS_PER_WG, NB_CMAX, SpvCounts, SpvDecParams, check, ptr, round_up, stream_ptr

N_HIDDEN_MIX = 256


@dataclass
class GroupCounts:

    X: torch.Tensor
    G: int
    col_off: int = 0
    resident: bool = False

    def __post_init__(self):
        self._xb = None
# ... 135 lines not shown
        t = self._ident.get(key)
        if t is None:
            t = self._ident[key] = torch.arange(B, dtype=torch.int32, device=self.device)
        return t


def gather_minibatches(items, nsplit: int, N1: int):
    lib = _abi.load()
    args = (_abi.SpvCsrGatherArgs * len(items))()
    out = []
    if not 0 < len(items) <= _abi.SPV_CSR_GATHER_MAXG:
        raise _abi.SpvError(f"gather_minibatches: 1 .. {_abi.SPV_CSR_GATHER_MAXG} groups per call")
    for a, (sc, rows, ws) in zip(args, items):
        if rows.dtype != torch.int32 or not rows.is_cuda or not rows.is_contiguous():
            raise _abi.SpvError("row index must be a contiguous int32 tensor in HBM")
        B, G = int(rows.numel()), sc.G
        ldx = round_up(G, 8)
        X = ws.get("csr_X", (B, ldx), torch.float32 if sc.dtype == _abi.SPV_COUNT_F32 else torch.int16)
        ldh = round_up(round_up(G, 96), 128)
        split = None
        if nsplit == 1:
            split = 0
        elif lib.spv_enc_fc1_fwd_uses_dma(B, G, N1, nsplit, 1, round_up(G, 64), 2 * ldh):
            split = 1
        xb = ws.get("csr_xb", (B, ldh if split == 0 else 2 * ldh), torch.int16) if split is not None else None
        lib_t = ws.get("csr_library", (B,), torch.float32) if split is not None else None
        a.indptr, a.cols, a.vals, a.n_rows, a.G, a.dtype, a.B = ptr(sc.indptr), ptr(sc.cols), ptr(sc.vals), sc.n_cells, G, sc.dtype, B
        a.rows, a.X, a.ldx = ptr(rows), ptr(X), ldx
        a.xb, a.ld_xb, a.xb_split, a.library = ptr(xb), (xb.shape[1] if xb is not None else 0), int(split or 0), ptr(lib_t)
        mb = GroupCounts(X, G, 0, resident=True)
        if split == 0:
            mb._xb = (xb, lib_t)
        elif split == 1:
            mb._xb_split = (xb, lib_t)
        out.append((mb, sc.identity_rows(B), B))
    _abi.call("spv_csr_gather", args, len(items), stream_ptr())
    return out


def image_token(*tensors) -> Tuple:
    return tuple((t.data_ptr(), t._version, tuple(t.shape)) for t in tensors)


_SIDE_STREAMS: Dict[Tuple, "torch.cuda.Stream"] = {}
SERIAL_STREAMS = os.environ.get("SPV_SERIAL_STREAMS", "auto") == "1"
SERIAL_AUTO = os.environ.get("SPV_SERIAL_STREAMS", "auto") == "auto"
SMALL_STEP_ELEMS = 4_000_000
_SMALL_STEP = False


def set_step_shape(B: int, G_max: int, n_groups: int) -> None:
    global _SMALL_STEP
    _SMALL_STEP = bool(n_groups == 2 and B * G_max <= SMALL_STEP_ELEMS)


def serial_streams() -> bool:
    return SERIAL_STREAMS or (SERIAL_AUTO and _SMALL_STEP and DEC_PAIR != "0")


def group_streams(device, n: int = 2, serial: Optional[bool] = None):
    dev = torch.device(device)
    out = [torch.cuda.current_stream(dev)]
    if serial_streams() if serial is None else serial:
        return out * n
    for i in range(1, n):
        key = (dev.index, i)
        if key not in _SIDE_STREAMS:
            _SIDE_STREAMS[key] = torch.cuda.Stream(device=dev)
        out.append(_SIDE_STREAMS[key])
    return out


def fork(streams) -> None:
    for st in streams[1:]:
        st.wait_stream(streams[0])


def join(streams) -> None:
    for st in streams[1:]:
        streams[0].wait_stream(st)


DEFER_JOIN = False

WM_LATE = os.environ.get("SPV_WM_LATE", "auto")
WM_LATE_MIN_G = 16384


def wm_late_for(G_max: int, grads_f32: bool) -> bool:
    if WM_LATE == "auto":
        return (not grads_f32) and G_max >= WM_LATE_MIN_G
    return WM_LATE != "0"



FC1_GROUPED = os.environ.get("SPV_FC1_GROUPED", "1") != "0"
LABEL_PRE = int(os.environ.get("SPV_LABEL_PRE", "-1"))
LABEL_PRE_MIN_B = 1024


def label_pre_for(B: int) -> int:
    return LABEL_PRE if LABEL_PRE >= 0 else (2 if B >= LABEL_PRE_MIN_B else 0)



DEC_PAIR = os.environ.get("SPV_DEC_PAIR", "auto")


def dec_pair_for(B: int, n_groups: int) -> bool:
    if n_groups != 2 or DEC_PAIR == "0":
        return False
    return True if DEC_PAIR == "1" else _SMALL_STEP


class DecSchedule(NamedTuple):

    serial: bool
    pair: bool
    wm_late: bool


def dec_schedule(B: int, Gs: Sequence[int], n_groups: int, grads_f32: bool) -> DecSchedule:
    return DecSchedule(bool(serial_streams()), bool(dec_pair_for(B, n_groups)), bool(wm_late_for(max(Gs), grads_f32)))


FC1_PAIR_SPLITS = os.environ.get("SPV_FC1_PAIR_SPLITS", "1") != "0"
GSPLIT_WANT = int(os.environ.get("SPV_GSPLIT_WANT", "512"))
FUSED_DZ = os.environ.get("SPV_FUSED_DZ", "1") != "0"
LINEAR_BWD = os.environ.get("SPV_LINEAR_BWD", "1") != "0"
TRUNK_FOLD = os.environ.get("SPV_TRUNK_FOLD", "1") != "0"
_PENDING: list = []
_PENDING_KEEP: list = []


def defer(stream, keep=()) -> None:
    if stream not in _PENDING:
        _PENDING.append(stream)
    _PENDING_KEEP.extend(keep)


def join_all_side_streams(device) -> None:
    dev = torch.device(device)
    cur = torch.cuda.current_stream(dev)
    capturing = torch.cuda.is_current_stream_capturing()
    for (idx, _i), st in _SIDE_STREAMS.items():
        if idx != dev.index or st is cur:
            continue
        if capturing:
            with torch.cuda.stream(st):
                if not torch.cuda.is_current_stream_capturing():
                    continue
        cur.wait_stream(st)


def join_pending(device=None) -> None:
    while _PENDING:
        st = _PENDING.pop()
        torch.cuda.current_stream(st.device if device is None else device).wait_stream(st)
    _PENDING_KEEP.clear()


def _pack(src: torch.Tensor, dst_hi: torch.Tensor, dst_lo: Optional[torch.Tensor], *, extra_col: Optional[torch.Tensor] = None,
          extra_one: bool = False, dst_row_off: int = 0, dst_col_off: int = 0, rows_cover: Optional[int] = None,
          cslot: Optional[int] = None) -> None:
    if src.dtype != torch.float32 or src.dim() != 2 or src.stride(1) != 1:
        raise _abi.SpvError("pack source must be fp32 [R][C] with unit column stride")
# ... 256 lines not shown
```

spvipes_amd/train.py:

```python
from __future__ import annotations

from typing import Dict, List, Optional, Sequence

import gc
import os

import torch
import torch.distributed as dist

from . import _abi
from .data import MinibatchSampler
from .module import spVIPESmodule
from .ops import GroupCounts


def kl_weight_at(epoch: int, step: int, n_epochs_kl_warmup: Optional[int], n_steps_kl_warmup: Optional[int],
                 max_kl_weight: float = 1.0, min_kl_weight: float = 0.0) -> float:
    slope = max_kl_weight - min_kl_weight
    if n_epochs_kl_warmup:
        if epoch < n_epochs_kl_warmup:
            return min_kl_weight + slope * (epoch / n_epochs_kl_warmup)
    elif n_steps_kl_warmup:
        if step < n_steps_kl_warmup:
            return min_kl_weight + slope * (step / n_steps_kl_warmup)
    return max_kl_weight


def default_max_epochs(n_obs: int) -> int:
    return int(min(round((20000 / n_obs) * 400), 400))


def sync_float_buffers(module: torch.nn.Module, world: int) -> None:
    if world <= 1:
        return
    bufs = [b for b in module.buffers() if b.is_floating_point() and b.numel()]
    if not bufs:
        return
    flat = torch.cat([b.detach().reshape(-1).to(torch.float32) for b in bufs])
    dist.all_reduce(flat, op=dist.ReduceOp.SUM)
    flat.div_(world)
    off = 0
    with torch.no_grad():
        for b in bufs:
            b.copy_(flat[off:off + b.numel()].view_as(b))
            off += b.numel()


class EarlyStopping:

    def __init__(self, patience: int, min_delta: float, world: int = 1, device=None):
        self.patience, self.min_delta, self.world, self.device = int(patience), float(min_delta), int(world), device
        self.best, self.bad_epochs = float("inf"), 0

    def reduced(self, value: float) -> float:
        if self.world <= 1:
            return float(value)
        t = torch.tensor([float(value)], dtype=torch.float64, device=self.device)
        dist.all_reduce(t, op=dist.ReduceOp.SUM)
        return float(t) / self.world

    def should_stop(self, value: float) -> bool:
        v = self.reduced(value)
        if v < self.best - self.min_delta:
            self.best, self.bad_epochs = v, 0
            return False
        self.bad_epochs += 1
        return self.bad_epochs >= self.patience


class FlatParams:

    def __init__(self, module: torch.nn.Module, late=None):
        named = [(n, p) for n, p in module.named_parameters() if p.requires_grad]
        if not named:
            raise ValueError("module has no trainable parameters")
        early = [p for n, p in named if late is None or not late(n)]
        params = early + [p for n, p in named if late is not None and late(n)]
        dev = params[0].device
        sizes = [(p.numel() + 3) // 4 * 4 for p in params]
        total = sum(sizes)
        self.flat = torch.zeros(total, dtype=torch.float32, device=dev)
        self.grad = torch.zeros(total, dtype=torch.float32, device=dev)
        self.split = sum(sizes[:len(early)])
        off = 0
        for p, n in zip(params, sizes):
            view = self.flat[off:off + p.numel()].view_as(p)
            view.copy_(p.data)
            p.data = view
            p.grad = self.grad[off:off + p.numel()].view_as(p)
            off += n
        self.params, self.numel = params, total

    def zero_grad(self):
        self.grad.zero_()


class HipAdam:

    def __init__(self, fp: FlatParams, lr=1e-3, betas=(0.9, 0.999), eps=0.01, weight_decay=1e-6):
        self.fp, self.lr, self.betas, self.eps, self.wd = fp, lr, betas, eps, weight_decay
        self.m = torch.zeros_like(fp.flat)
        self.v = torch.zeros_like(fp.flat)
        self.t = 0
        self.t_dev = torch.zeros((), dtype=torch.int64, device=fp.flat.device)

    def step(self, grad_scale: float = 1.0, images=None, counter=None):
        self.t += 1
        self.launch(grad_scale, images, counter)

    def launch(self, grad_scale: float = 1.0, images=None, counter=None):
        b1, b2 = self.betas
        n_img = len(images) if images is not None else 0
        _abi.call("spv_adam_step_images", _abi.ptr(self.fp.flat), _abi.ptr(self.fp.grad), _abi.ptr(self.m), _abi.ptr(self.v),
                  self.fp.numel, self.lr, b1, b2, self.eps, self.wd, 1.0, 1.0,
                  grad_scale, images if n_img else None, n_img, _abi.ptr(counter), _abi.ptr(self.t_dev), float(b1), float(b2), _abi.stream_ptr())
        _abi.call("spv_counter_bump", _abi.ptr(self.t_dev), _abi.stream_ptr())


class Trainer:

    def __init__(self, module: spVIPESmodule, counts: Sequence[GroupCounts], labels: Optional[Sequence[torch.Tensor]] = None,
                 components: Optional[Sequence[torch.Tensor]] = None, lr: float = 1e-3, eps: float = 0.01,
                 weight_decay: float = 1e-6, n_epochs_kl_warmup: Optional[int] = 400, n_steps_kl_warmup: Optional[int] = None,
                 overlap_allreduce: Optional[bool] = None, batch_codes: Optional[Sequence[torch.Tensor]] = None, world: Optional[int] = None):
        self.module, self.counts, self.labels, self.components = module, list(counts), labels, components
        self.batch_codes = None
        if getattr(module, "n_cov", 0):
            if batch_codes is None or len(batch_codes) != len(self.counts):
                raise ValueError(f"the module was built with n_batch = {module.n_batch}: pass batch_codes (one code per cell and group)")
            self.batch_codes = [b.flatten().to(device=counts[0].device, dtype=torch.int32).contiguous() for b in batch_codes]
            for g, b in enumerate(self.batch_codes):
                if b.numel() and not bool(((b >= 0) & (b < module.n_cov)).all()):
                    raise ValueError(f"batch codes of group {g} must lie in [0, n_batch = {module.n_batch})")
        for what, codes in (("labels", labels), ("cluster components", components)):
            if codes is None:
                continue
            for g, l in enumerate(codes):
                lf = l.flatten().to(torch.float32)
                if lf.numel() and not bool(((lf >= 0) & (lf < _abi.POE_LMAX) & (lf == lf.floor())).all()):
                    raise ValueError(f"{what} of group {g} must be integral codes in [0, {_abi.POE_LMAX})")
                n_comp = getattr(module, "n_components", None)
                if what == "cluster components" and module.n_groups > 2 and n_comp is not None and lf.numel() and float(lf.max()) >= n_comp:
                    raise ValueError(f"cluster components of group {g} must be codes in [0, n_components = {n_comp})")
        self.device = counts[0].device
        self.fp = FlatParams(module, late=lambda name: name.startswith("encoder_"))
        self.opt = HipAdam(self.fp, lr=lr, eps=eps, weight_decay=weight_decay)
        self.n_epochs_kl_warmup, self.n_steps_kl_warmup = n_epochs_kl_warmup, n_steps_kl_warmup
        self._pg_world = dist.get_world_size() if dist.is_available() and dist.is_initialized() else 1
        self.world = self._pg_world if world is None else int(world)
        self.overlap = (self.world > 1) if overlap_allreduce is None else bool(overlap_allreduce)
        self.global_step, self.epoch = 0, 0
        if self.DEVICE_RNG:
            rank = dist.get_rank() if self.world > 1 else 0
            module.enable_device_rng(self.device, key=(int(torch.initial_seed()) * 0x9E3779B97F4A7C15 + 1) & 0xFFFFFFFFFFFFFFFF, counter0=rank << 40)
        self.graph = self.graph2 = None
        self.last_outputs = None
        self.history: Dict[str, List[float]] = {"train_loss": [], "elbo_train": [], "reconstruction_loss_train": [], "kl_local_train": []}

    IMAGES_BY_ADAM = os.environ.get("SPV_ADAM_IMAGES", "1") != "0"
    ZERO_GRADS_EACH_STEP = os.environ.get("SPV_ZERO_GRADS", "0") != "0"
    DEVICE_RNG = os.environ.get("SPV_DEVICE_RNG", "1") != "0"
    MULTI_GATHER = os.environ.get("SPV_MULTI_GATHER", "1") != "0"
    ADAM_IN_GRAPH = os.environ.get("SPV_ADAM_IN_GRAPH", "1") != "0"

    def _image_specs(self):
        from . import ops
        from .dec_ops import KMP

        m = self.module
        out = []
        for g in range(m.n_groups):
            ws = m._workspace(g, self.device)
            ep, es = m.encoders[g]["private"], m.encoders[g]["shared"]
            H, G = ep.fc1.weight.shape
            N1 = 2 * H
            bn = 32 if N1 <= 32 else (128 if N1 <= 128 else 256)
            img = ops._bf16_image(ws, "fc1_W", ops.round_up(N1, bn), ops.round_up(G, 64), False)[0]
            out.append((ws, "fc1_W", img, [(ep.fc1.weight, 0, 0), (es.fc1.weight, H, 0)], (ep.fc1.weight, es.fc1.weight)))
            dec = m.decoders[g]
            Wm, bm = dec.mixture.linear.weight, dec.mixture.linear.bias
            img = ops._bf16_image(ws, "dec_Wm", ops.round_up(G, 256), KMP, False)[0]
            out.append((ws, "dec_Wm", img, [(Wm, 0, 0), (bm, 0, Wm.shape[1])], (Wm, bm)))
        return out

    def _build_image_plan(self):
        if not self.IMAGES_BY_ADAM or self.module.nsplit != 1 or getattr(self.module, "n_cov", 0):
            self._img_specs, self._img_plan = [], None
            return
        from . import ops
        specs = self._image_specs()
        offs = {}
        for p_ in self.fp.params:
            offs[id(p_)] = (p_.data_ptr() - self.fp.flat.data_ptr()) // 4
        descs = []
        for ws, key, img, parts, _tok in specs:
            for par, row_off, col_off in parts:
                if id(par) not in offs:
                    self._img_specs, self._img_plan = [], None
                    return
                d = _abi.SpvAdamImage()
                d.begin, d.count = offs[id(par)], par.numel()
                d.cols = par.shape[1] if par.dim() == 2 else 1
                d.row_off, d.col_off, d.ld, d.dst = row_off, col_off, img.shape[1], _abi.ptr(img)
                d.fmt, d.scale = (_abi.IMAGE_F16, ops.fc1_w_scale()) if key == "fc1_W" else (_abi.IMAGE_BF16, 1.0)
                descs.append(d)
        if not descs or len(descs) > _abi.ADAM_MAX_IMAGES:
            self._img_specs, self._img_plan = [], None
            return
        self._img_specs, self._img_plan = specs, (_abi.SpvAdamImage * len(descs))(*descs)

    def _images_are_fresh(self) -> bool:
        from .ops import image_token
        if getattr(self, "_flat_version", None) != self.fp.flat._version:
            return False
        return all(ws.fresh.get(key) == image_token(*tok) for ws, key, _img, _parts, tok in self._img_specs)

    def _mark_images_fresh(self) -> None:
        from .ops import image_token
        for ws, key, _img, _parts, tok in self._img_specs:
            ws.fresh[key] = image_token(*tok)
        self._flat_version = self.fp.flat._version

    def parameters_changed(self) -> None:
        for ws, key, _img, _parts, _tok in getattr(self, "_img_specs", []):
            ws.fresh.pop(key, None)

    def _ensure_images(self) -> None:
        from . import ops
        if getattr(self, "_img_plan", "unset") == "unset":
            self._build_image_plan()
        if self._img_plan is None or self._images_are_fresh():
            return
        for ws, key, img, parts, _tok in self._img_specs:
            if key == "fc1_W":
                (wp, _, _), (wsh, H, _) = parts
                ops._pack_fc1_weights(wp, wsh, img, None, H)
            else:
                (Wm, _, _), (bm, _, _) = parts
                ops._pack(Wm, img, None, extra_col=bm)
        self._mark_images_fresh()

    def minibatch(self, rows: Sequence[torch.Tensor]):
        out = []
        need_idx = bool(getattr(self.module, "use_transport_plan", False))
        if self.labels is not None and getattr(self, "_labels_f32", None) is None:
            self._labels_f32 = [l.flatten().to(torch.float32).contiguous() for l in self.labels]
        lab = None
        if self.labels is not None:
            if self.MULTI_GATHER and all(r.dtype == torch.int32 and r.is_cuda and r.is_contiguous() for r in rows):
                lab = [torch.empty(r.numel(), dtype=torch.float32, device=r.device) for r in rows]
                _abi.gather_u32([(self._labels_f32[g], r, lab[g]) for g, r in enumerate(rows)])
            else:
                lab = [self._labels_f32[g].index_select(0, r) for g, r in enumerate(rows)]
        for g, r in enumerate(rows):
            d = {"counts": self.counts[g], "rows": r, "groups": None, "batch": None}
            if self.batch_codes is not None:
                d["batch"] = self.batch_codes[g].index_select(0, r)
            d["indices"] = r.to(torch.float32).unsqueeze(1) if need_idx else None
            if lab is not None:
                d["labels"] = lab[g].unsqueeze(1)
            if self.components is not None:
                d["processed_transport_labels"] = self.components[g][r.long()].unsqueeze(1)
            out.append(d)
        return tuple(out)

    def _forward_backward(self, rows, kl_weight, noise=None):
        from . import nn_ops, ops

        if self.ZERO_GRADS_EACH_STEP:
            self.fp.grad.zero_()
        self.module.split_backward = self.overlap
        try:
            inf, gen, lo = self.module(self.minibatch(rows), inference_kwargs=({"noise": noise} if noise is not None else None),
                                       loss_kwargs={"kl_weight": kl_weight})
            self.last_outputs = (inf, gen)
        finally:
            self.module.split_backward = False
        nn_ops.GRAD_SINK = True
        ops.DEFER_JOIN = True
        try:
            one = getattr(self, "_one", None)
            if one is None or one.device != lo.loss.device:
                one = self._one = torch.ones((), dtype=torch.float32, device=lo.loss.device)
            cut = self.module._cut
            if cut is not None:
                extra = ([p for n, p in self.module.named_parameters() if p.requires_grad and not n.startswith("encoder_")]
                         if getattr(self.module, "n_cov", 0) else [])
                grads = torch.autograd.grad(lo.loss, list(cut[1]) + extra, grad_outputs=one, allow_unused=True)
                self._cut_grads = grads[:len(cut[1])]
                for p, g in zip(extra, grads[len(cut[1]):]):
                    if g is not None:
                        p.grad.copy_(g)
            else:
                lo.loss.backward(gradient=one)
        finally:
            nn_ops.GRAD_SINK = False
            ops.DEFER_JOIN = False
            ops.join_pending()
            ops.join_all_side_streams(self.device)
        return lo

    def _backward_encoders(self):
        from . import nn_ops, ops

        outs, _cut = self.module._cut
        pairs = [(o, g) for o, g in zip(outs, self._cut_grads) if g is not None and o.requires_grad]
        nn_ops.GRAD_SINK = True
        ops.DEFER_JOIN = True
        try:
            torch.autograd.backward([o for o, _ in pairs], [g for _, g in pairs])
        finally:
            nn_ops.GRAD_SINK = False
            ops.DEFER_JOIN = False
            ops.join_pending()
            ops.join_all_side_streams(self.device)
        self.module._cut = self._cut_grads = None

    def capture(self, rows: Sequence[torch.Tensor], warmup: int = 3) -> None:
        from . import ops

        if self.graph is not None:
            return
        self._ensure_images()
        self._static_rows = [r.clone() for r in rows]
        self._klw = torch.ones((), dtype=torch.float32, device=self.device)
        self._klw_host = 1.0
        side = torch.cuda.Stream(device=self.device)
        side.wait_stream(torch.cuda.current_stream())
        with torch.cuda.stream(side):
            for _ in range(warmup):
                self._forward_backward(self._static_rows, self._klw)
                if self.overlap:
                    self._backward_encoders()
        torch.cuda.current_stream().wait_stream(side)
        mode = {}
        if self._pg_world > 1:
            torch.cuda.synchronize(self.device)
            mode = {"capture_error_mode": "thread_local"}
        keep = os.environ.get("SPV_GRAPH_KEEP") == "1"
        g = torch.cuda.CUDAGraph(keep_graph=True) if keep else torch.cuda.CUDAGraph()
        self._adam_in_graph = bool(self.ADAM_IN_GRAPH and self.world == 1 and not self.overlap)
        gc_was_on = gc.isenabled()
        gc.collect()
        gc.disable()
        try:
            with torch.cuda.graph(g, **mode):
                self._static_lo = self._forward_backward(self._static_rows, self._klw)
                if self._adam_in_graph:
                    self.opt.launch(grad_scale=1.0, images=self._img_plan, counter=getattr(self.module, "_rng_counter", None))
            if keep:
                g.instantiate()
            self.graph = g
            if self.overlap:
                g2 = torch.cuda.CUDAGraph(keep_graph=True) if keep else torch.cuda.CUDAGraph()
                with torch.cuda.graph(g2, pool=g.pool(), **mode):
                    self._backward_encoders()
                if keep:
                    g2.instantiate()
                self.graph2 = g2
        finally:
            if gc_was_on:
                gc.enable()

    def step(self, rows: Sequence[torch.Tensor], kl_weight: Optional[float] = None, noise=None, optimizer_step: bool = True):
        if noise is not None and self.graph is not None:
            raise ValueError("injected noise needs an eager step (the captured graph draws its own)")
        if kl_weight is None:
            kl_weight = kl_weight_at(self.epoch, self.global_step, self.n_epochs_kl_warmup, self.n_steps_kl_warmup)
        self._ensure_images()
        if self.graph is not None:
            if self.MULTI_GATHER and all(r.dtype == torch.int32 and r.is_cuda and r.is_contiguous() and r.numel() == s.numel() for s, r in zip(self._static_rows, rows)):
                _abi.gather_u32([(r, None, s) for s, r in zip(self._static_rows, rows)])
            else:
                for s, r in zip(self._static_rows, rows):
                    s.copy_(r)
            if float(kl_weight) != self._klw_host:
                self._klw.fill_(float(kl_weight))
                self._klw_host = float(kl_weight)
            self.graph.replay()
            lo = self._static_lo
        else:
            lo = self._forward_backward(rows, kl_weight, noise)
        timed = self.world > 1
        if timed:
            if getattr(self, "_ev_ar", None) is None:
                self._ev_ar = (torch.cuda.Event(enable_timing=True), torch.cuda.Event(enable_timing=True))
        if self.overlap:
            split = self.fp.split
            w1 = dist.all_reduce(self.fp.grad[:split], op=dist.ReduceOp.SUM, async_op=True) if self.world > 1 else None
            if self.graph is not None:
                self.graph2.replay()
            else:
                self._backward_encoders()
            if self.world > 1:
                self._ev_ar[0].record()
                w2 = dist.all_reduce(self.fp.grad[split:], op=dist.ReduceOp.SUM, async_op=True)
                w1.wait()
                w2.wait()
                self._ev_ar[1].record()
        elif self.world > 1:
            self._ev_ar[0].record()
            dist.all_reduce(self.fp.grad, op=dist.ReduceOp.SUM)
            self._ev_ar[1].record()
        if self.graph is not None and getattr(self, "_adam_in_graph", False):
            if not optimizer_step:
                raise ValueError("this trainer's captured graph contains the optimiser step: use an eager step for optimizer_step=False")
            self.opt.t += 1
            self.global_step += 1
        elif optimizer_step:
            plan = getattr(self, "_img_plan", None)
            if plan is not None and not self._images_are_fresh():
                plan = None
                self.parameters_changed()
            self.opt.step(grad_scale=1.0 / self.world, images=plan, counter=getattr(self.module, "_rng_counter", None))
            self.global_step += 1
        return lo

    def last_allreduce_exposed_ms(self) -> float:
        if self.world <= 1 or getattr(self, "_ev_ar", None) is None:
            return 0.0
        self._ev_ar[1].synchronize()
        return float(self._ev_ar[0].elapsed_time(self._ev_ar[1]))

    @torch.no_grad()
    def validation_metrics(self, sampler: MinibatchSampler):
        B = sampler.batch_size
        nb = [len(v) // B for v in sampler.val_idx]
        if not nb or min(nb) == 0:
            return None
        was_training = self.module.training
        self.module.eval()
        val = [torch.as_tensor(v, dtype=torch.int32, device=self.device) for v in sampler.val_idx]
        acc = None
        for step in range(max(nb)):
            rows = [v[(step % n) * B:(step % n + 1) * B].contiguous() for v, n in zip(val, nb)]
            _, _, lo = self.module(self.minibatch(rows), loss_kwargs={"kl_weight": 1.0})
            rec = lo.reconstruction_loss_mean
            cur = torch.stack([lo.loss, rec, lo.loss - rec])
            acc = cur if acc is None else acc + cur
        self.module.train(was_training)
        tot, rec, kl = (float(v) / max(nb) for v in acc.cpu())
        return {"elbo_validation": rec + kl, "reconstruction_loss_validation": rec, "kl_local_validation": kl, "validation_loss": tot}

    def fit(self, sampler: MinibatchSampler, max_epochs: int, log_every: int = 0, use_graph: bool = True, early_stopping: bool = False,
            early_stopping_patience: int = 45, early_stopping_min_delta: float = 0.0, check_val_every_n_epoch: Optional[int] = None):
        if check_val_every_n_epoch is None:
            check_val_every_n_epoch = 1 if early_stopping else 0
        if early_stopping and (not sampler.val_idx or min(len(v) // sampler.batch_size for v in sampler.val_idx) == 0):
            raise ValueError("early_stopping needs at least one full validation batch per group (train_size < 1 / validation_size > 0)")
        for k in ("elbo_validation", "reconstruction_loss_validation", "kl_local_validation", "validation_loss"):
            self.history.setdefault(k, [])
        stopper = EarlyStopping(early_stopping_patience, early_stopping_min_delta, self.world, self.device) if early_stopping else None
        self.module.train()
        for ep in range(max_epochs):
            self.epoch = ep
            acc = None
            for rows in sampler.epoch():
                if use_graph and self.graph is None:
                    self.capture(rows)
                klw = kl_weight_at(self.epoch, self.global_step, self.n_epochs_kl_warmup, self.n_steps_kl_warmup)
                lo = self.step(rows, kl_weight=klw)
                if log_every and (self.global_step % log_every == 0):
                    loss = lo.loss.detach()
                    rec = lo.reconstruction_loss_mean if lo.reconstruction_loss_mean is not None else sum(v.mean() for v in lo.reconstruction_loss.values())
                    if klw > 1e-12:
                        kl = (loss - rec) / klw
                    else:
                        kl = sum(v.detach().mean() for v in lo.kl_local.values())
                    cur = torch.stack([loss, rec.detach(), kl, torch.ones_like(loss)])
                    acc = cur if acc is None else acc + cur
            if acc is not None:
                tot, rec, kl, n = (float(v) for v in acc.cpu())
                self.history["train_loss"].append(tot / n)
                self.history["reconstruction_loss_train"].append(rec / n)
                self.history["kl_local_train"].append(kl / n)
                self.history["elbo_train"].append((rec + kl) / n)
            if check_val_every_n_epoch and (ep + 1) % check_val_every_n_epoch == 0:
                sync_float_buffers(self.module, self.world)
                vm = self.validation_metrics(sampler)
                if vm is not None:
                    for k, v in vm.items():
                        self.history[k].append(v)
                    if stopper is not None and stopper.should_stop(vm["elbo_validation"]):
                        self.stopped_epoch = ep
                        break
        sync_float_buffers(self.module, self.world)
        self.module.eval()
        return self.history
```

Baseline: 6.338 million.

## Fuse slab reduction of weight-mixing gradients with Adam update and skip them later

Adds a kernel that reduces the per-slab gradient partials for selected weight-mixing parameters and applies the Adam update, including the bf16/f16 image write, in the same pass. The main Adam kernel gets skip ranges so it does not update those parameters again. The aim is to avoid writing the reduced gradient and then rereading it along with p/m/v in the separate optimizer pass. The cost is index remapping in the main Adam loop and a more complex ordering dependency inside the captured graph. The path is limited to single-device, non-pair schedules.

```diff
diff --git a/include/spvipes_hip.h b/include/spvipes_hip.h
--- a/include/spvipes_hip.h
+++ b/include/spvipes_hip.h
@@ -358,9 +358,13 @@
   float scale; int32_t _pad;
 } spv_adam_image;
 
+#define SPV_ADAM_MAX_SKIP 8
+typedef struct spv_adam_range { int64_t begin, count; } spv_adam_range;
+
 int spv_adam_step_images(float* p, const float* g, float* m, float* v, int64_t n, float lr, float beta1, float beta2, float eps,
                          float weight_decay, float bc1, float bc2, float grad_scale, const spv_adam_image* images, int32_t n_images,
-                         int64_t* step_counter, const int64_t* t_dev, double beta1_d, double beta2_d, void* stream);
+                         const spv_adam_range* skip, int32_t n_skip, int64_t* step_counter, const int64_t* t_dev, double beta1_d,
+                         double beta2_d, void* stream);
 
 typedef struct spv_gather_prob { const uint32_t* src; const int32_t* idx; uint32_t* dst; int64_t count; } spv_gather_prob;
 int spv_gather_u32(const spv_gather_prob* probs, int32_t nprob, void* stream);
@@ -572,6 +576,12 @@
 typedef struct spv_reduce_batch { spv_reduce_prob p[SPV_MAXR]; int32_t nprob; } spv_reduce_batch;
 int spv_reduce_slabs(const spv_reduce_batch* b, void* stream);
 
+#define SPV_MAXRA 8
+typedef struct spv_reduce_adam_prob { spv_reduce_prob r; float* p; float* m; float* v; spv_adam_image img; } spv_reduce_adam_prob;
+typedef struct spv_reduce_adam_batch { spv_reduce_adam_prob p[SPV_MAXRA]; int32_t nprob; } spv_reduce_adam_batch;
+int spv_reduce_slabs_adam(const spv_reduce_adam_batch* b, float lr, float beta1, float beta2, float eps, float weight_decay,
+                          float bc1, float bc2, float grad_scale, const int64_t* t_dev, double beta1_d, double beta2_d, void* stream);
+
 int spv_loss_assemble(const float* rec0, const float* rec1, const float* w, const float* const* kl, int32_t nkl, int32_t B,
                       const float* kl_weight, float* loss, float* rec_sum, float* gkl, void* stream);
 
diff --git a/spvipes_amd/_abi.py b/spvipes_amd/_abi.py
--- a/spvipes_amd/_abi.py
+++ b/spvipes_amd/_abi.py
@@ -152,6 +152,22 @@
 class SpvAdamImage(C.Structure):
     _fields_ = [("begin", C.c_int64), ("count", C.c_int64), ("cols", C.c_int32), ("row_off", C.c_int32), ("col_off", C.c_int32), ("fmt", C.c_int32),
                 ("ld", C.c_int64), ("dst", C.c_void_p), ("scale", C.c_float), ("_pad", C.c_int32)]
+
+
+ADAM_MAX_SKIP = 8
+SPV_MAXRA = 8
+
+
+class SpvAdamRange(C.Structure):
+    _fields_ = [("begin", C.c_int64), ("count", C.c_int64)]
+
+
+class SpvReduceAdamProb(C.Structure):
+    _fields_ = [("r", SpvReduceProb), ("p", C.c_void_p), ("m", C.c_void_p), ("v", C.c_void_p), ("img", SpvAdamImage)]
+
+
+class SpvReduceAdamBatch(C.Structure):
+    _fields_ = [("p", SpvReduceAdamProb * SPV_MAXRA), ("nprob", C.c_int32)]
 
 
 class SpvPoeCompArgs(C.Structure):
@@ -427,8 +443,10 @@
     "spv_loss_assemble": (C.c_int, [C.c_void_p, C.c_void_p, C.c_void_p, C.POINTER(C.c_void_p), C.c_int32, C.c_int32, C.c_void_p, C.c_void_p,
                                     C.c_void_p, C.c_void_p, C.c_void_p]),
     "spv_adam_step_images": (C.c_int, [C.c_void_p, C.c_void_p, C.c_void_p, C.c_void_p, C.c_int64, C.c_float, C.c_float, C.c_float, C.c_float,
-                                       C.c_float, C.c_float, C.c_float, C.c_float, C.c_void_p, C.c_int32, C.c_void_p, C.c_void_p, C.c_double, C.c_double,
-                                       C.c_void_p]),
+                                       C.c_float, C.c_float, C.c_float, C.c_float, C.c_void_p, C.c_int32, C.c_void_p, C.c_int32, C.c_void_p, C.c_void_p,
+                                       C.c_double, C.c_double, C.c_void_p]),
+    "spv_reduce_slabs_adam": (C.c_int, [C.POINTER(SpvReduceAdamBatch), C.c_float, C.c_float, C.c_float, C.c_float, C.c_float, C.c_float, C.c_float,
+                                        C.c_float, C.c_void_p, C.c_double, C.c_double, C.c_void_p]),
     "spv_gather_u32": (C.c_int, [C.c_void_p, C.c_int32, C.c_void_p]),
     "spv_randn": (C.c_int, [C.c_void_p, C.c_int64, C.c_void_p, C.c_uint64, C.c_void_p]),
     "spv_counter_bump": (C.c_int, [C.c_void_p, C.c_void_p]),
diff --git a/spvipes_amd/build.py b/spvipes_amd/build.py
--- a/spvipes_amd/build.py
+++ b/spvipes_amd/build.py
@@ -10,7 +10,7 @@
 LIBDIR = os.path.join(HERE, "_lib")
 LIB = os.path.join(LIBDIR, "libspvipes_hip.so")
 SOURCES = ["spv_abi.hip"]
-HEADERS = ["spv_common.h", "spv_gemm.h", "spv_fc1.h", "spv_dec_gemm.h", "spv_decoder.h", "spv_dec_expected.h", "spv_dec_sample.h", "spv_dec_sample_stats.h", "spv_dec_expected_stats.h", "spv_de.h", "spv_de_median.h", "spv_count_stats.h", "spv_knn.h", "spv_pair_scan.h", "spv_ot.h", "spv_ot_segments.h", "spv_silhouette.h", "spv_small.h", "spv_poe_n.h", os.path.join("..", "..", "include", "spvipes_hip.h")]
+HEADERS = ["spv_common.h", "spv_adam.h", "spv_gemm.h", "spv_fc1.h", "spv_dec_gemm.h", "spv_decoder.h", "spv_dec_expected.h", "spv_dec_sample.h", "spv_dec_sample_stats.h", "spv_dec_expected_stats.h", "spv_de.h", "spv_de_median.h", "spv_count_stats.h", "spv_knn.h", "spv_pair_scan.h", "spv_ot.h", "spv_ot_segments.h", "spv_silhouette.h", "spv_small.h", "spv_poe_n.h", os.path.join("..", "..", "include", "spvipes_hip.h")]
 
 
 FLAGS = [
diff --git a/spvipes_amd/csrc/spv_abi.hip b/spvipes_amd/csrc/spv_abi.hip
--- a/spvipes_amd/csrc/spv_abi.hip
+++ b/spvipes_amd/csrc/spv_abi.hip
@@ -1247,26 +1247,20 @@
 __global__ void adam_kernel(float* __restrict__ p, const float* __restrict__ g, float* __restrict__ m, float* __restrict__ v,
                             long n, float lr, float b1, float b2, float eps, float wd, float bc1, float bc2, float gscale) {
   const long stride = (long)gridDim.x * blockDim.x * 4;
-  const float step = lr / bc1, isq = rsqrtf(bc2);
+  const AdamStep a = adam_prologue(lr, b1, b2, eps, wd, bc1, bc2, gscale, nullptr, 0.0, 0.0);
   for (long i = ((long)blockIdx.x * blockDim.x + threadIdx.x) * 4; i < n; i += stride) {
     if (i + 4 <= n) {
       f4v pp = *reinterpret_cast<f4v*>(p + i), gg = *reinterpret_cast<const f4v*>(g + i);
       f4v mm = *reinterpret_cast<f4v*>(m + i), vv = *reinterpret_cast<f4v*>(v + i);
 #pragma unroll
       for (int j = 0; j < 4; ++j) {
-        const float gr = gg[j] * gscale + wd * pp[j];
-        mm[j] = b1 * mm[j] + (1.f - b1) * gr;
-        vv[j] = b2 * vv[j] + (1.f - b2) * gr * gr;
-        pp[j] -= step * mm[j] / (sqrtf(vv[j]) * isq + eps);
+        float pj = pp[j], mj = mm[j], vj = vv[j];
+        adam_update(pj, gg[j], mj, vj, a);
+        pp[j] = pj; mm[j] = mj; vv[j] = vj;
       }
       *reinterpret_cast<f4v*>(p + i) = pp; *reinterpret_cast<f4v*>(m + i) = mm; *reinterpret_cast<f4v*>(v + i) = vv;
     } else {
-      for (long k = i; k < n; ++k) {
-        const float gr = g[k] * gscale + wd * p[k];
-        m[k] = b1 * m[k] + (1.f - b1) * gr;
-        v[k] = b2 * v[k] + (1.f - b2) * gr * gr;
-        p[k] -= step * m[k] / (sqrtf(v[k]) * isq + eps);
-      }
+      for (long k = i; k < n; ++k) adam_update(p[k], g[k], m[k], v[k], a);
     }
   }
 }
@@ -1328,41 +1322,34 @@
 }
 
 struct AdamImages { int n; spv_adam_image img[SPV_ADAM_MAX_IMAGES]; };
+struct AdamSkips { int n; long begin[SPV_ADAM_MAX_SKIP], count[SPV_ADAM_MAX_SKIP]; };
 
 __global__ void adam_images_kernel(float* __restrict__ p, const float* __restrict__ g, float* __restrict__ m, float* __restrict__ v,
-                                   long n, float lr, float b1, float b2, float eps, float wd, float bc1, float bc2, float gscale, AdamImages im,
-                                   long long* step_counter, const long long* t_dev, double b1d, double b2d) {
+                                   long n_kept, float lr, float b1, float b2, float eps, float wd, float bc1, float bc2, float gscale, AdamImages im,
+                                   AdamSkips sk, long long* step_counter, const long long* t_dev, double b1d, double b2d) {
   if (step_counter && blockIdx.x == 0 && threadIdx.x == 0) *step_counter += 1;
-  if (t_dev) {
-    long long e = *t_dev + 1;
-    double r1 = 1.0, r2 = 1.0, x1 = b1d, x2 = b2d;
-    while (e > 0) { if (e & 1) { r1 *= x1; r2 *= x2; } x1 *= x1; x2 *= x2; e >>= 1; }
-    bc1 = (float)(1.0 - r1); bc2 = (float)(1.0 - r2);
-  }
+  const AdamStep a = adam_prologue(lr, b1, b2, eps, wd, bc1, bc2, gscale, t_dev, b1d, b2d);
   const long stride = (long)gridDim.x * blockDim.x * 4;
-  const float step = lr / bc1, isq = rsqrtf(bc2);
-  for (long i = ((long)blockIdx.x * blockDim.x + threadIdx.x) * 4; i < n; i += stride) {
+  for (long ik = ((long)blockIdx.x * blockDim.x + threadIdx.x) * 4; ik < n_kept; ik += stride) {
     float out[4];
-    const int cnt = (i + 4 <= n) ? 4 : (int)(n - i);
+    const int cnt = (ik + 4 <= n_kept) ? 4 : (int)(n_kept - ik);
+    long i = ik;
+    for (int d = 0; d < sk.n; ++d) i += i >= sk.begin[d] ? sk.count[d] : 0;
     if (cnt == 4) {
       f4v pp = *reinterpret_cast<f4v*>(p + i), gg = *reinterpret_cast<const f4v*>(g + i);
       f4v mm = *reinterpret_cast<f4v*>(m + i), vv = *reinterpret_cast<f4v*>(v + i);
 #pragma unroll
       for (int j = 0; j < 4; ++j) {
-        const float gr = gg[j] * gscale + wd * pp[j];
-        mm[j] = b1 * mm[j] + (1.f - b1) * gr;
-        vv[j] = b2 * vv[j] + (1.f - b2) * gr * gr;
-        pp[j] -= step * mm[j] / (sqrtf(vv[j]) * isq + eps);
-        out[j] = pp[j];
+        float pj = pp[j], mj = mm[j], vj = vv[j];
+        adam_update(pj, gg[j], mj, vj, a);
+        pp[j] = pj; mm[j] = mj; vv[j] = vj;
+        out[j] = pj;
       }
       *reinterpret_cast<f4v*>(p + i) = pp; *reinterpret_cast<f4v*>(m + i) = mm; *reinterpret_cast<f4v*>(v + i) = vv;
     } else {
       for (int j = 0; j < cnt; ++j) {
         const long k = i + j;
-        const float gr = g[k] * gscale + wd * p[k];
-        m[k] = b1 * m[k] + (1.f - b1) * gr;
-        v[k] = b2 * v[k] + (1.f - b2) * gr * gr;
-        p[k] -= step * m[k] / (sqrtf(v[k]) * isq + eps);
+        adam_update(p[k], g[k], m[k], v[k], a);
         out[j] = p[k];
       }
     }
@@ -1370,29 +1357,24 @@
       const spv_adam_image& q = im.img[d];
       const long k0 = i - q.begin;
       if (k0 + cnt <= 0 || k0 >= q.count) continue;
-      const unsigned cols = (unsigned)q.cols;
-      unsigned r = (unsigned)k0 / cols, c = (unsigned)k0 - r * cols;
-      uint16_t* dst = q.dst + ((long)r + q.row_off) * q.ld + q.col_off;
-      const bool half = q.fmt == SPV_IMAGE_F16;
-      if (cnt == 4 && k0 + 4 <= q.count && c + 4 <= cols && (((reinterpret_cast<uintptr_t>(dst + c)) & 7) == 0)) {
-        typedef __attribute__((ext_vector_type(4))) unsigned short us4;
-        *reinterpret_cast<us4*>(dst + c) = half ? us4{f2h(out[0] * q.scale), f2h(out[1] * q.scale), f2h(out[2] * q.scale), f2h(out[3] * q.scale)}
-                                                : us4{f2bf(out[0]), f2bf(out[1]), f2bf(out[2]), f2bf(out[3])};
-      } else {
-        for (int j = 0; j < cnt && k0 + j < q.count; ++j) {
-          dst[c] = half ? f2h(out[j] * q.scale) : f2bf(out[j]);
-          if (++c == cols) { c = 0; dst += q.ld; }
-        }
-      }
+      adam_image_store(q, k0, cnt, out);
       break;
     }
   }
 }
 
+static bool adam_image_ok(const spv_adam_image& q) {
+  return q.dst && q.count > 0 && q.cols > 0 && q.ld >= q.cols + q.col_off && q.row_off >= 0 && q.col_off >= 0 && q.count < (1L << 31) &&
+         (q.fmt == SPV_IMAGE_BF16 || (q.fmt == SPV_IMAGE_F16 && q.scale > 0.f));
+}
+
 extern "C" int spv_adam_step_images(float* p, const float* g, float* m, float* v, int64_t n, float lr, float beta1, float beta2, float eps,
                                     float weight_decay, float bc1, float bc2, float grad_scale, const spv_adam_image* images, int32_t n_images,
-                                    int64_t* step_counter, const int64_t* t_dev, double beta1_d, double beta2_d, void* stream) {
-  if (!p || !g || !m || !v || n < 0 || n_images < 0 || n_images > SPV_ADAM_MAX_IMAGES || (n_images && !images)) return fail(SPV_ERR_ARG, "spv_adam_step_images: bad arguments%s");
+                                    const spv_adam_range* skip, int32_t n_skip, int64_t* step_counter, const int64_t* t_dev, double beta1_d,
+                                    double beta2_d, void* stream) {
+  if (!p || !g || !m || !v || n < 0 || n_images < 0 || n_images > SPV_ADAM_MAX_IMAGES || (n_images && !images) || n_skip < 0 ||
+      n_skip > SPV_ADAM_MAX_SKIP || (n_skip && !skip))
+    return fail(SPV_ERR_ARG, "spv_adam_step_images: bad arguments%s");
   if (n == 0) return SPV_OK;
   if ((reinterpret_cast<uintptr_t>(p) | reinterpret_cast<uintptr_t>(g) | reinterpret_cast<uintptr_t>(m) | reinterpret_cast<uintptr_t>(v)) & 15)
     return fail(SPV_ERR_ARG, "spv_adam_step_images: buffers must be 16-byte aligned%s");
@@ -1400,17 +1382,56 @@
   im.n = n_images;
   for (int d = 0; d < n_images; ++d) {
     const spv_adam_image& q = images[d];
-    if (!q.dst || q.begin < 0 || (q.begin & 3) || q.count <= 0 || q.begin + q.count > n || q.cols <= 0 || q.ld < q.cols + q.col_off || q.row_off < 0 || q.col_off < 0 ||
-        q.count >= (1L << 31) || (q.fmt != SPV_IMAGE_BF16 && q.fmt != SPV_IMAGE_F16) || (q.fmt == SPV_IMAGE_F16 && !(q.scale > 0.f)))
+    if (!adam_image_ok(q) || q.begin < 0 || (q.begin & 3) || q.begin + q.count > n)
       return fail(SPV_ERR_ARG, "spv_adam_step_images: bad image descriptor%s");
     im.img[d] = q;
   }
-  long blocks = (n / 4 + 255) / 256;
+  AdamSkips sk{};
+  sk.n = n_skip;
+  long n_kept = n, end = 0;
+  for (int d = 0; d < n_skip; ++d) {
+    const spv_adam_range& r = skip[d];
+    if (r.begin < end || (r.begin & 3) || r.count <= 0 || r.begin + r.count > n || ((r.count & 3) && r.begin + r.count != n))
+      return fail(SPV_ERR_ARG, "spv_adam_step_images: bad skip range%s");
+    sk.begin[d] = r.begin; sk.count[d] = r.count;
+    end = r.begin + r.count;
+    n_kept -= r.count;
+  }
+  if (n_kept == 0) {
+    return step_counter ? spv_counter_bump(step_counter, stream) : SPV_OK;
+  }
+  long blocks = (n_kept / 4 + 255) / 256;
   if (blocks > 2048) blocks = 2048;
   if (blocks < 1) blocks = 1;
-  hipLaunchKernelGGL(adam_images_kernel, dim3((unsigned)blocks), dim3(256), 0, (hipStream_t)stream, p, g, m, v, (long)n, lr, beta1, beta2, eps,
-                     weight_decay, bc1, bc2, grad_scale, im, (long long*)step_counter, (const long long*)t_dev, beta1_d, beta2_d);
+  hipLaunchKernelGGL(adam_images_kernel, dim3((unsigned)blocks), dim3(256), 0, (hipStream_t)stream, p, g, m, v, n_kept, lr, beta1, beta2, eps,
+                     weight_decay, bc1, bc2, grad_scale, im, sk, (long long*)step_counter, (const long long*)t_dev, beta1_d, beta2_d);
   return launch_status("spv_adam_step_images");
+}
+
+extern "C" int spv_reduce_slabs_adam(const spv_reduce_adam_batch* b, float lr, float beta1, float beta2, float eps, float weight_decay,
+                                     float bc1, float bc2, float grad_scale, const int64_t* t_dev, double beta1_d, double beta2_d, void* stream) {
+  if (!b || b->nprob <= 0 || b->nprob > SPV_MAXRA) return fail(SPV_ERR_ARG, "spv_reduce_slabs_adam: bad batch%s");
+  ReduceAdamArgs a{};
+  a.nprob = b->nprob;
+  long blocks = 1;
+  for (int i = 0; i < b->nprob; ++i) {
+    const spv_reduce_adam_prob& q = b->p[i];
+    const spv_reduce_prob& r = q.r;
+    if (!r.src || !r.dst || r.nslabs <= 0 || r.nslabs > RED_FEW_MAX || r.rows <= 0 || r.cols <= 0 || r.ld_src < r.col_off + r.cols || r.col_off < 0 ||
+        (long)r.rows * r.cols >= (1l << 31) || r.ld_dst != r.cols || r.accumulate || r.exp_scale || !q.p || !q.m || !q.v)
+      return fail(SPV_ERR_ARG, "spv_reduce_slabs_adam: bad problem%s");
+    if (q.img.dst && (!adam_image_ok(q.img) || q.img.cols != r.cols || q.img.count != (long)r.rows * r.cols))
+      return fail(SPV_ERR_ARG, "spv_reduce_slabs_adam: bad image descriptor%s");
+    a.p[i] = q;
+    long t = ((long)r.rows * r.cols + 255) / 256;
+    if (t > 8192) t = 8192;
+    a.nblk[i] = (unsigned)t;
+    if (t > blocks) blocks = t;
+  }
+  a.lr = lr; a.b1 = beta1; a.b2 = beta2; a.eps = eps; a.wd = weight_decay; a.bc1 = bc1; a.bc2 = bc2; a.gscale = grad_scale;
+  a.t_dev = (const long long*)t_dev; a.b1d = beta1_d; a.b2d = beta2_d;
+  hipLaunchKernelGGL(reduce_adam_fused_kernel, dim3((unsigned)blocks, b->nprob), dim3(256), 0, (hipStream_t)stream, a);
+  return launch_status("spv_reduce_slabs_adam");
 }
 
 extern "C" int spv_adam_step(float* p, const float* g, float* m, float* v, int64_t n, float lr, float beta1, float beta2,
diff --git a/spvipes_amd/csrc/spv_adam.h b/spvipes_amd/csrc/spv_adam.h
--- /dev/null
+++ b/spvipes_amd/csrc/spv_adam.h
@@ -0,0 +1,49 @@
+#pragma once
+#include "../../include/spvipes_hip.h"
+#include "spv_common.h"
+
+namespace spv {
+
+struct AdamStep { float b1, b2, eps, wd, gscale, step, isq; };
+
+__device__ __forceinline__ AdamStep adam_prologue(float lr, float b1, float b2, float eps, float wd, float bc1, float bc2, float gscale,
+                                                  const long long* t_dev, double b1d, double b2d) {
+  if (t_dev) {
+    long long e = *t_dev + 1;
+    double r1 = 1.0, r2 = 1.0, x1 = b1d, x2 = b2d;
+    while (e > 0) { if (e & 1) { r1 *= x1; r2 *= x2; } x1 *= x1; x2 *= x2; e >>= 1; }
+    bc1 = (float)(1.0 - r1); bc2 = (float)(1.0 - r2);
+  }
+  AdamStep a;
+  a.b1 = b1; a.b2 = b2; a.eps = eps; a.wd = wd; a.gscale = gscale;
+  a.step = lr / bc1; a.isq = rsqrtf(bc2);
+  return a;
+}
+
+__device__ __forceinline__ void adam_update(float& p, float g, float& m, float& v, const AdamStep& a) {
+  const float gr = __fmaf_rn(g, a.gscale, __fmul_rn(a.wd, p));
+  m = __fmaf_rn(a.b1, m, __fmul_rn(1.f - a.b1, gr));
+  v = __fmaf_rn(a.b2, v, __fmul_rn(__fmul_rn(1.f - a.b2, gr), gr));
+  p -= __fmul_rn(a.step, m) / __fmaf_rn(sqrtf(v), a.isq, a.eps);
+}
+
+__device__ __forceinline__ uint16_t adam_image_word(const spv_adam_image& q, float x) {
+  return q.fmt == SPV_IMAGE_F16 ? f2h(x * q.scale) : f2bf(x);
+}
+
+__device__ __forceinline__ void adam_image_store(const spv_adam_image& q, long k0, int cnt, const float (&out)[4]) {
+  const unsigned cols = (unsigned)q.cols;
+  unsigned r = (unsigned)k0 / cols, c = (unsigned)k0 - r * cols;
+  uint16_t* dst = q.dst + ((long)r + q.row_off) * q.ld + q.col_off;
+  if (cnt == 4 && k0 + 4 <= q.count && c + 4 <= cols && (((reinterpret_cast<uintptr_t>(dst + c)) & 7) == 0)) {
+    typedef __attribute__((ext_vector_type(4))) unsigned short us4;
+    *reinterpret_cast<us4*>(dst + c) = us4{adam_image_word(q, out[0]), adam_image_word(q, out[1]), adam_image_word(q, out[2]), adam_image_word(q, out[3])};
+  } else {
+    for (int j = 0; j < cnt && k0 + j < q.count; ++j) {
+      dst[c] = adam_image_word(q, out[j]);
+      if (++c == cols) { c = 0; dst += q.ld; }
+    }
+  }
+}
+
+}
diff --git a/spvipes_amd/csrc/spv_small.h b/spvipes_amd/csrc/spv_small.h
--- a/spvipes_amd/csrc/spv_small.h
+++ b/spvipes_amd/csrc/spv_small.h
@@ -1,6 +1,7 @@
 #pragma once
 #include "../../include/spvipes_hip.h"
 #include "spv_common.h"
+#include "spv_adam.h"
 
 namespace spv {
 
@@ -1613,6 +1614,47 @@
   }
 }
 
+struct ReduceAdamArgs {
+  spv_reduce_adam_prob p[SPV_MAXRA]; int nprob;
+  unsigned nblk[SPV_MAXRA];
+  float lr, b1, b2, eps, wd, bc1, bc2, gscale; const long long* t_dev; double b1d, b2d;
+};
+template <int NS>
+__device__ __forceinline__ void reduce_adam_few(const spv_reduce_adam_prob& q, unsigned nblk, float alpha, const AdamStep& a) {
+  const spv_reduce_prob& rq = q.r;
+  const unsigned cols = (unsigned)rq.cols, total = (unsigned)rq.rows * cols;
+  for (unsigned e = blockIdx.x * 256u + threadIdx.x; e < total; e += nblk * 256u) {
+    const unsigned r = e / cols, c = e - r * cols;
+    const float* s = rq.src + (long)r * rq.ld_src + rq.col_off + c;
+    float t[NS];
+#pragma unroll
+    for (int k = 0; k < NS; ++k) t[k] = s[(long)k * rq.slab_stride];
+    float p = q.p[e], m = q.m[e], v = q.v[e];
+    const float g = __fmul_rn(reduce_ordered_sum<NS>(t), alpha);
+    rq.dst[e] = g;
+    adam_update(p, g, m, v, a);
+    q.p[e] = p; q.m[e] = m; q.v[e] = v;
+    if (q.img.dst) q.img.dst[((long)r + q.img.row_off) * q.img.ld + q.img.col_off + c] = adam_image_word(q.img, p);
+  }
+}
+__global__ __launch_bounds__(256) void reduce_adam_fused_kernel(ReduceAdamArgs b) {
+  const spv_reduce_adam_prob& q = b.p[blockIdx.y];
+  const unsigned nblk = b.nblk[blockIdx.y];
+  if (blockIdx.x >= nblk) return;
+  const float alpha = *(q.r.alpha ? q.r.alpha : &g_spv_one);
+  const AdamStep a = adam_prologue(b.lr, b.b1, b.b2, b.eps, b.wd, b.bc1, b.bc2, b.gscale, b.t_dev, b.b1d, b.b2d);
+  switch (q.r.nslabs) {
+    case 1: reduce_adam_few<1>(q, nblk, alpha, a); break;
+    case 2: reduce_adam_few<2>(q, nblk, alpha, a); break;
+    case 3: reduce_adam_few<3>(q, nblk, alpha, a); break;
+    case 4: reduce_adam_few<4>(q, nblk, alpha, a); break;
+    case 5: reduce_adam_few<5>(q, nblk, alpha, a); break;
+    case 6: reduce_adam_few<6>(q, nblk, alpha, a); break;
+    case 7: reduce_adam_few<7>(q, nblk, alpha, a); break;
+    default: reduce_adam_few<8>(q, nblk, alpha, a); break;
+  }
+}
+
 __global__ __launch_bounds__(1024) void loss_assemble_kernel(const float* rec0, const float* rec1, const float* w, const float* kl0,
                                                              const float* kl1, const float* kl2, const float* kl3, int B,
                                                              const float* kl_weight, float* loss, float* rec_sum, float* gkl) {
diff --git a/spvipes_amd/dec_ops.py b/spvipes_amd/dec_ops.py
--- a/spvipes_amd/dec_ops.py
+++ b/spvipes_amd/dec_ops.py
@@ -64,6 +64,21 @@
 def _run_red(b: SpvReduceBatch) -> None:
     if b.nprob:
         _abi.call("spv_reduce_slabs", C.byref(b), stream_ptr())
+
+
+def _reduce_adam(b: SpvReduceBatch, params, targets) -> bool:
+    fa = _ops.WM_ADAM
+    if fa is None or not b.nprob or b.nprob != len(params) or b.nprob > _abi.SPV_MAXRA or len(fa.taken) + b.nprob > _abi.ADAM_MAX_SKIP:
+        return False
+    ba = _abi.SpvReduceAdamBatch()
+    ba.nprob = b.nprob
+    for i in range(b.nprob):
+        q, r = ba.p[i], b.p[i]
+        if r.nslabs > 8 or r.accumulate or r.exp_scale or r.ld_dst != r.cols or not fa.fill(q, params[i], targets[i]):
+            return False
+        q.r = r
+    fa.launch(ba, params)
+    return True
 
 
 def _zsplit_args(B: int, Bp: int, n_p: int, n_s: int, n_m: int, sl, lat, zcat, Am_img, Aps_img) -> SpvZsplitArgs:
@@ -636,7 +651,9 @@
                     a = wm_slabs[g] if pair else st.gemm_a()
                     _add_red(red3, a, st.csp_m, G * KMP, KMP, G, KM - 1, pg[g][10][0], KM - 1, alpha=g_loss)
                     _add_red(red3, a, st.csp_m, G * KMP, KMP, G, 1, pg[g][11][0], 1, col_off=KM - 1, alpha=g_loss)
-                _run_red(red3)
+                if sched.pair or not _reduce_adam(red3, [par[g][j] for g in range(NG) for j in (10, 11)],
+                                                   [pg[g][j][0] for g in range(NG) for j in (10, 11)]):
+                    _run_red(red3)
             if _ops.DEFER_JOIN:
                 _ops.defer(side, [g_loss])
             else:
diff --git a/spvipes_amd/ops.py b/spvipes_amd/ops.py
--- a/spvipes_amd/ops.py
+++ b/spvipes_amd/ops.py
@@ -241,6 +241,7 @@
 
 
 DEFER_JOIN = False
+WM_ADAM = None
 
 WM_LATE = os.environ.get("SPV_WM_LATE", "auto")
 WM_LATE_MIN_G = 16384
diff --git a/spvipes_amd/train.py b/spvipes_amd/train.py
--- a/spvipes_amd/train.py
+++ b/spvipes_amd/train.py
@@ -2,6 +2,7 @@
 
 from typing import Dict, List, Optional, Sequence
 
+import ctypes as C
 import gc
 import os
 
@@ -104,17 +105,56 @@
         self.t = 0
         self.t_dev = torch.zeros((), dtype=torch.int64, device=fp.flat.device)
 
-    def step(self, grad_scale: float = 1.0, images=None, counter=None):
+    def step(self, grad_scale: float = 1.0, images=None, counter=None, skip=()):
         self.t += 1
-        self.launch(grad_scale, images, counter)
-
-    def launch(self, grad_scale: float = 1.0, images=None, counter=None):
+        self.launch(grad_scale, images, counter, skip)
+
+    def launch(self, grad_scale: float = 1.0, images=None, counter=None, skip=()):
         b1, b2 = self.betas
         n_img = len(images) if images is not None else 0
+        ranges = (_abi.SpvAdamRange * len(skip))(*[_abi.SpvAdamRange(b, c) for b, c in skip]) if skip else None
         _abi.call("spv_adam_step_images", _abi.ptr(self.fp.flat), _abi.ptr(self.fp.grad), _abi.ptr(self.m), _abi.ptr(self.v),
                   self.fp.numel, self.lr, b1, b2, self.eps, self.wd, 1.0, 1.0,
-                  grad_scale, images if n_img else None, n_img, _abi.ptr(counter), _abi.ptr(self.t_dev), float(b1), float(b2), _abi.stream_ptr())
+                  grad_scale, images if n_img else None, n_img, ranges, len(skip), _abi.ptr(counter), _abi.ptr(self.t_dev), float(b1), float(b2),
+                  _abi.stream_ptr())
         _abi.call("spv_counter_bump", _abi.ptr(self.t_dev), _abi.stream_ptr())
+
+
+class FusedWmAdam:
+
+    def __init__(self, opt: HipAdam, images: Optional[dict] = None):
+        self.opt, self.images, self.taken = opt, images or {}, []
+
+    def fill(self, q, param: torch.Tensor, target: torch.Tensor) -> bool:
+        fp = self.opt.fp
+        delta, n = param.data_ptr() - fp.flat.data_ptr(), param.numel()
+        if param.dtype != torch.float32 or not param.is_contiguous() or delta < 0 or delta % 16 or delta // 4 + n > fp.numel:
+            return False
+        off = delta // 4
+        if target.data_ptr() != fp.grad.data_ptr() + delta:
+            return False
+        q.p, q.m, q.v = fp.flat.data_ptr() + 4 * off, self.opt.m.data_ptr() + 4 * off, self.opt.v.data_ptr() + 4 * off
+        img = self.images.get(off)
+        if img is not None:
+            q.img = img
+        return True
+
+    def launch(self, batch, params) -> None:
+        b1, b2 = self.opt.betas
+        _abi.call("spv_reduce_slabs_adam", C.byref(batch), self.opt.lr, b1, b2, self.opt.eps, self.opt.wd, 1.0, 1.0, 1.0,
+                  _abi.ptr(self.opt.t_dev), float(b1), float(b2), _abi.stream_ptr())
+        fp = self.opt.fp
+        for p_ in params:
+            self.taken.append(((p_.data_ptr() - fp.flat.data_ptr()) // 4, (p_.numel() + 3) // 4 * 4))
+
+    def ranges(self):
+        out = []
+        for b, c in sorted(self.taken):
+            if out and out[-1][0] + out[-1][1] == b:
+                out[-1] = (out[-1][0], out[-1][1] + c)
+            else:
+                out.append((b, c))
+        return out
 
 
 class Trainer:
@@ -162,6 +202,7 @@
     DEVICE_RNG = os.environ.get("SPV_DEVICE_RNG", "1") != "0"
     MULTI_GATHER = os.environ.get("SPV_MULTI_GATHER", "1") != "0"
     ADAM_IN_GRAPH = os.environ.get("SPV_ADAM_IN_GRAPH", "1") != "0"
+    FUSED_WM_ADAM = os.environ.get("SPV_FUSED_WM_ADAM", "1") != "0"
 
     def _image_specs(self):
         from . import ops
@@ -264,7 +305,13 @@
             out.append(d)
         return tuple(out)
 
-    def _forward_backward(self, rows, kl_weight, noise=None):
+    def _fused_wm_adam(self, images) -> Optional[FusedWmAdam]:
+        if not self.FUSED_WM_ADAM or self.world != 1:
+            return None
+        by_begin = {d.begin: d for d in images} if images is not None else {}
+        return FusedWmAdam(self.opt, by_begin)
+
+    def _forward_backward(self, rows, kl_weight, noise=None, fused: Optional[FusedWmAdam] = None):
         from . import nn_ops, ops
 
         if self.ZERO_GRADS_EACH_STEP:
@@ -278,6 +325,7 @@
             self.module.split_backward = False
         nn_ops.GRAD_SINK = True
         ops.DEFER_JOIN = True
+        ops.WM_ADAM = fused
         try:
             one = getattr(self, "_one", None)
             if one is None or one.device != lo.loss.device:
@@ -296,6 +344,7 @@
         finally:
             nn_ops.GRAD_SINK = False
             ops.DEFER_JOIN = False
+            ops.WM_ADAM = None
             ops.join_pending()
             ops.join_all_side_streams(self.device)
         return lo
@@ -345,9 +394,11 @@
         gc.disable()
         try:
             with torch.cuda.graph(g, **mode):
-                self._static_lo = self._forward_backward(self._static_rows, self._klw)
+                fused = self._fused_wm_adam(self._img_plan) if self._adam_in_graph else None
+                self._static_lo = self._forward_backward(self._static_rows, self._klw, fused=fused)
                 if self._adam_in_graph:
-                    self.opt.launch(grad_scale=1.0, images=self._img_plan, counter=getattr(self.module, "_rng_counter", None))
+                    self.opt.launch(grad_scale=1.0, images=self._img_plan, counter=getattr(self.module, "_rng_counter", None),
+                                    skip=fused.ranges() if fused is not None else ())
             if keep:
                 g.instantiate()
             self.graph = g
@@ -368,6 +419,7 @@
         if kl_weight is None:
             kl_weight = kl_weight_at(self.epoch, self.global_step, self.n_epochs_kl_warmup, self.n_steps_kl_warmup)
         self._ensure_images()
+        fused = None
         if self.graph is not None:
             if self.MULTI_GATHER and all(r.dtype == torch.int32 and r.is_cuda and r.is_contiguous() and r.numel() == s.numel() for s, r in zip(self._static_rows, rows)):
                 _abi.gather_u32([(r, None, s) for s, r in zip(self._static_rows, rows)])
@@ -380,7 +432,12 @@
             self.graph.replay()
             lo = self._static_lo
         else:
-            lo = self._forward_backward(rows, kl_weight, noise)
+            if optimizer_step:
+                plan = getattr(self, "_img_plan", None)
+                if plan is not None and not self._images_are_fresh():
+                    plan = None
+                fused = self._fused_wm_adam(plan)
+            lo = self._forward_backward(rows, kl_weight, noise, fused=fused)
         timed = self.world > 1
         if timed:
             if getattr(self, "_ev_ar", None) is None:
@@ -412,7 +469,8 @@
             if plan is not None and not self._images_are_fresh():
                 plan = None
                 self.parameters_changed()
-            self.opt.step(grad_scale=1.0 / self.world, images=plan, counter=getattr(self.module, "_rng_counter", None))
+            self.opt.step(grad_scale=1.0 / self.world, images=plan, counter=getattr(self.module, "_rng_counter", None),
+                          skip=fused.ranges() if fused is not None else ())
             self.global_step += 1
         return lo
 
```

Result: faster. 6.431 million (median of 6 runs) (+1.5%).
